# victorca25/traiNNer

Measured on NVIDIA B200. Metric: hr_pixels_per_sec, higher is better.
Workload: dtype bf16

## Files before the change

include/trainner_b200.h:

```cpp
#ifndef TRAINNER_B200_H_
#define TRAINNER_B200_H_

#include <stddef.h>
#include <stdint.h>

#ifdef __cplusplus
extern "C" {
#endif

typedef void* b200_stream_t;

#define B200_MAX_TAPS 16

typedef struct {
  int32_t n, h_in, w_in;
  int32_t cx, cin_off, cin;
  int32_t h_out, w_out;
  int32_t h_buf, w_buf, cy;
  int32_t cout_off, cout;
  int32_t ntaps;
  int8_t tap_dy[B200_MAX_TAPS], tap_dx[B200_MAX_TAPS], tap_w[B200_MAX_TAPS];
  int32_t in_stride, in_off_y, in_off_x;
  int32_t out_mul_y, out_off_y, out_mul_x, out_off_x;
  int32_t upsample2x;
  int32_t w_taps, w_cout_pad, w_cin_pad;
  float alpha;
  int32_t act;
  float slope;
  float beta1, beta2;
  int32_t res_nch;
  int32_t res1_c, res1_coff, res2_c, res2_coff;
  int32_t accumulate;
  int32_t mask_c, mask_coff, mask_lo, mask_hi;
  float mask_slope;
  int32_t parity_classes;
} b200_conv_desc;

int b200_conv_igemm(const b200_conv_desc* d, const void* x, const void* w_packed, const float* bias,
                    const void* res1, const void* res2, const void* mask, void* y,
                    b200_stream_t stream);
int b200_conv_igemm_stat_rows(const b200_conv_desc* d);
int b200_conv_igemm_stats(const b200_conv_desc* d, const void* x, const void* w_packed, const float* bias,
                          void* y, float* stat_part, b200_stream_t stream);

typedef struct {
  int32_t n, h, w;
  int32_t cx, cin_off, cin;
  int32_t cx2, cin2_off, cin2;
  int32_t cy, cout_off, cout;
  int8_t tap_dy[9], tap_dx[9], tap_w[9];
  int32_t out_mode;
  int32_t w_taps, w_cout_pad, w_cin_pad;
  float alpha;
  int32_t act;
  float slope;
  float beta1, beta2;
  int32_t res_nch, res1_c, res1_coff, res2_c, res2_coff;
  int32_t accumulate;
  int32_t mask_c, mask_coff, mask_lo, mask_hi;
  float mask_slope;
} b200_flat_desc;

int b200_conv3x3_flat(const b200_flat_desc* d, const void* x, const void* x2, const void* w_packed,
                      const float* bias, const void* res1, const void* res2, const void* mask, void* y,
                      b200_stream_t stream);

int b200_pad_copy(void* dst_flat, int32_t dst_c, int32_t dst_coff, const void* src_dense, int32_t src_c,
                  int32_t src_coff, int32_t n, int32_t h, int32_t w, int32_t c, b200_stream_t stream);
int b200_unpad_add(void* dst_dense, int32_t dst_c, const void* src_flat, int32_t src_c, int32_t src_coff,
                   const void* add_dense, int32_t add_c, int32_t n, int32_t h, int32_t w, int32_t c,
                   b200_stream_t stream);

typedef struct {
  void* out;
  const float* bias;
  const void* mask;
  const void* res1;
  const void* res2;
  int32_t out_c, out_coff, mask_c, mask_coff, res1_c, res1_coff, res2_c, res2_coff;
  float alpha, beta1, beta2, slope, mask_slope;
  int32_t act;
  int32_t pad_[2];
} b200_chain_stage;

typedef struct {
  int32_t n_total, img0, n;
  int32_t h, w;
  int32_t cx, x_coff;
  int32_t n_blocks;
  int32_t flip_taps;
} b200_chain_desc;

int b200_rdb_chain_geometry(int32_t n, int32_t h, int32_t w, int32_t* n_cta, int64_t* ll_bytes);
int b200_rdb_chain(const b200_chain_desc* d, const void* x0, const void* const* w_stage,
                   const b200_chain_stage* table_dev, void* ll_buf, int64_t ll_bytes, uint32_t* epoch_dev,
                   b200_stream_t stream);

typedef struct {
  int32_t n, h_in, w_in, cx, x_coff, cin;
  int32_t h_out, w_out, cdy, dy_coff, cout;
  int32_t kh, kw, stride, pad;
  float scale;
} b200_wgrad_desc;

int b200_conv_wgrad(const b200_wgrad_desc* d, const void* x, const void* dy, float* dw,
                    float* dbias, b200_stream_t stream);

typedef struct {
  float* dw[5];
  float scale5;
  int32_t pad_;
} b200_wgrad_rdb_entry;

int b200_tensor_map_bytes(void);
int b200_wgrad_rdb_make_maps(void* maps_host, int32_t n_rdb, const void* const* x_ptrs,
                             const void* const* g_ptrs, const void* const* do_ptrs,
                             const int32_t* do_pitch, int32_t n, int32_t h, int32_t w, int32_t c);
int64_t b200_wgrad_rdb_ws_bytes(int32_t n_rdb, int32_t n, int32_t h, int32_t w);
int b200_wgrad_rdb(const void* maps_dev, const b200_wgrad_rdb_entry* entries_dev, int32_t n_rdb,
                   int32_t n, int32_t h, int32_t w, int32_t nf, int32_t gc, void* workspace,
                   int64_t ws_bytes, b200_stream_t stream);

typedef struct {
  const void* src;
  float* dst;
  int64_t npix;
  int32_t pitch, coff, c;
  float scale;
} b200_colsum_entry;

int b200_colsum_multi(const b200_colsum_entry* table_dev, int32_t count, b200_stream_t stream);

typedef struct {
  const float* src;
  void* dst;
  int32_t cout, cin, taps, rows_pad, cols_pad, mode;
  int32_t co_mul, co_off;
} b200_pack_entry;

int b200_pack_weights(const b200_pack_entry* table_dev, int32_t count, int32_t max_elems,
                      b200_stream_t stream);

typedef struct {
  const float* src;
  void* dst;
  int32_t cout, cin, taps, ci_off, n_rows, rows_pad, cols_pad, col_off;
  float scale;
  int32_t row_off;
  int32_t mode;
  int32_t pad_;
} b200_packcat_entry;

int b200_pack_cat(const b200_packcat_entry* table_dev, int32_t count, int32_t max_elems,
                  b200_stream_t stream);

int b200_conv3x3_thin_to_wide(const float* x, const float* w_oihw, const float* bias, void* y,
                              int32_t n, int32_t h, int32_t w, int32_t cs, int32_t cw, int32_t cy,
                              int32_t y_coff, int32_t transpose_w, const float* mean,
                              const float* std, int32_t act, float slope, const void* mask,
                              int32_t mask_c, int32_t mask_coff, float mask_slope,
                              b200_stream_t stream);
int b200_conv3x3_wide_to_thin(const void* x, const float* w_oihw, const float* bias, float* y,
                              int32_t n, int32_t h, int32_t w, int32_t cw, int32_t cx, int32_t x_coff,
                              int32_t cs, int32_t transpose_w, const float* inv_std, float out_scale,
                              b200_stream_t stream);
int b200_conv3x3_thin_wgrad(const float* thin, const void* wide, float* dw, float* dbias_wide,
                            float* dbias_thin, int32_t n, int32_t h, int32_t w, int32_t cs,
                            int32_t cw, int32_t cwide_buf, int32_t wide_coff, int32_t wide_is_out,
                            const float* mean, const float* std, b200_stream_t stream);

int b200_bn_stats_finalize(const void* z, float* stats, float* mean_invstd, float* running_mean,
                           float* running_var, int64_t npix, int32_t c, float momentum, float eps,
                           b200_stream_t stream);
typedef struct {
  const float* stats;
  float* mean_invstd;
  float* running_mean;
  float* running_var;
  int64_t npix;
  int32_t c;
  float momentum, eps;
  int32_t pad_;
} b200_bn_finalize_entry;
int b200_bn_finalize_multi(const b200_bn_finalize_entry* table_dev, int32_t count, int32_t c_max,
                           b200_stream_t stream);
int b200_bn_partials_finalize(const float* part, int32_t rows, float* stats, float* mean_invstd,
                              float* running_mean, float* running_var, int64_t npix, int32_t c, float momentum,
                              float eps, b200_stream_t stream);
int b200_bn_apply_lrelu(const void* z, const float* mean_invstd, const float* gamma,
                        const float* beta, void* a, int64_t npix, int32_t c, float slope,
                        b200_stream_t stream);
int b200_bn_bwd_reduce(const void* z, const void* da, const float* mean_invstd,
                       const float* gamma, const float* beta, float* sums, float* dgamma, float* dbeta,
                       int64_t npix, int32_t c, float slope, b200_stream_t stream);
int b200_bn_bwd_apply(const void* z, const void* da, const float* mean_invstd, const float* gamma,
                      const float* beta, const float* sums, void* dz, int64_t npix, int32_t c, float slope,
                      int32_t use_batch_stats, b200_stream_t stream);

int b200_maxpool2x2(const void* x, void* y, int32_t n, int32_t h, int32_t w, int32_t c,
                    b200_stream_t stream);
int b200_maxpool2x2_bwd(const void* x, const void* dy, void* dx, int32_t n, int32_t h, int32_t w,
                        int32_t c, b200_stream_t stream);

int b200_sumpool2x2_mask(const void* dy, const void* mask_up, void* dx, int32_t n, int32_t h,
                         int32_t w, int32_t c, float slope, b200_stream_t stream);
int b200_pixel_shuffle2(const void* z, void* out, int32_t n, int32_t h, int32_t w, int32_t c,
                        int32_t act, float slope, b200_stream_t stream);
int b200_pixel_unshuffle2(const void* dout, void* dz, int32_t n, int32_t h, int32_t w, int32_t c,
                          b200_stream_t stream);

int b200_l1_loss_f32(const float* a, const float* b, float* loss_out, float* grad_a, int64_t numel,
                     float weight, b200_stream_t stream);
int b200_l1_loss_bf16(const void* a, const void* b, float* loss_out, void* grad_a, int64_t numel,
                      float weight, b200_stream_t stream);

int b200_lrelu_mask_mul(const void* g, const void* y, void* out, int64_t numel, float slope,
                        b200_stream_t stream);
int b200_nchw_f32_to_nhwc_bf16(const float* x, void* y, int32_t n, int32_t c, int32_t h, int32_t w,
                               int32_t cy, int32_t y_coff, b200_stream_t stream);
int b200_nhwc_bf16_to_nchw_f32(const void* x, float* y, int32_t n, int32_t c, int32_t h, int32_t w,
                               int32_t cx, int32_t x_coff, b200_stream_t stream);

const char* b200_last_error(void);
int b200_version(void);
int b200_device_ok(void);
int64_t b200_launch_count(void);

#ifdef __cplusplus
}
#endif
#endif
```

trainner_b200/_lib.py:

```python
import ctypes as C
import os

_HERE = os.path.dirname(os.path.abspath(__file__))
LIB_PATH = os.path.join(_HERE, "libtrainner_b200.so")

MAX_TAPS = 16


class ConvDesc(C.Structure):
    _fields_ = [
        ("n", C.c_int32), ("h_in", C.c_int32), ("w_in", C.c_int32),
        ("cx", C.c_int32), ("cin_off", C.c_int32), ("cin", C.c_int32),
        ("h_out", C.c_int32), ("w_out", C.c_int32),
        ("h_buf", C.c_int32), ("w_buf", C.c_int32), ("cy", C.c_int32),
        ("cout_off", C.c_int32), ("cout", C.c_int32),
        ("ntaps", C.c_int32),
        ("tap_dy", C.c_int8 * MAX_TAPS), ("tap_dx", C.c_int8 * MAX_TAPS), ("tap_w", C.c_int8 * MAX_TAPS),
        ("in_stride", C.c_int32), ("in_off_y", C.c_int32), ("in_off_x", C.c_int32),
        ("out_mul_y", C.c_int32), ("out_off_y", C.c_int32), ("out_mul_x", C.c_int32), ("out_off_x", C.c_int32),
        ("upsample2x", C.c_int32),
        ("w_taps", C.c_int32), ("w_cout_pad", C.c_int32), ("w_cin_pad", C.c_int32),
        ("alpha", C.c_float), ("act", C.c_int32), ("slope", C.c_float),
        ("beta1", C.c_float), ("beta2", C.c_float),
        ("res_nch", C.c_int32),
        ("res1_c", C.c_int32), ("res1_coff", C.c_int32), ("res2_c", C.c_int32), ("res2_coff", C.c_int32),
        ("accumulate", C.c_int32),
        ("mask_c", C.c_int32), ("mask_coff", C.c_int32), ("mask_lo", C.c_int32), ("mask_hi", C.c_int32),
        ("mask_slope", C.c_float),
        ("parity_classes", C.c_int32),
    ]


class FlatDesc(C.Structure):
    _fields_ = [
        ("n", C.c_int32), ("h", C.c_int32), ("w", C.c_int32),
        ("cx", C.c_int32), ("cin_off", C.c_int32), ("cin", C.c_int32),
        ("cx2", C.c_int32), ("cin2_off", C.c_int32), ("cin2", C.c_int32),
        ("cy", C.c_int32), ("cout_off", C.c_int32), ("cout", C.c_int32),
        ("tap_dy", C.c_int8 * 9), ("tap_dx", C.c_int8 * 9), ("tap_w", C.c_int8 * 9),
        ("out_mode", C.c_int32),
        ("w_taps", C.c_int32), ("w_cout_pad", C.c_int32), ("w_cin_pad", C.c_int32),
        ("alpha", C.c_float), ("act", C.c_int32), ("slope", C.c_float),
        ("beta1", C.c_float), ("beta2", C.c_float),
        ("res_nch", C.c_int32), ("res1_c", C.c_int32), ("res1_coff", C.c_int32),
        ("res2_c", C.c_int32), ("res2_coff", C.c_int32),
        ("accumulate", C.c_int32),
        ("mask_c", C.c_int32), ("mask_coff", C.c_int32), ("mask_lo", C.c_int32), ("mask_hi", C.c_int32),
        ("mask_slope", C.c_float),
    ]


class WgradDesc(C.Structure):
    _fields_ = [
        ("n", C.c_int32), ("h_in", C.c_int32), ("w_in", C.c_int32), ("cx", C.c_int32),
        ("x_coff", C.c_int32), ("cin", C.c_int32),
        ("h_out", C.c_int32), ("w_out", C.c_int32), ("cdy", C.c_int32), ("dy_coff", C.c_int32),
        ("cout", C.c_int32),
        ("kh", C.c_int32), ("kw", C.c_int32), ("stride", C.c_int32), ("pad", C.c_int32),
        ("scale", C.c_float),
    ]


class WgradRdbEntry(C.Structure):
    _fields_ = [("dw", C.c_void_p * 5), ("scale5", C.c_float), ("pad_", C.c_int32)]


class ColsumEntry(C.Structure):
    _fields_ = [("src", C.c_void_p), ("dst", C.c_void_p), ("npix", C.c_int64),
                ("pitch", C.c_int32), ("coff", C.c_int32), ("c", C.c_int32), ("scale", C.c_float)]


class BnFinalizeEntry(C.Structure):
    _fields_ = [("stats", C.c_void_p), ("mean_invstd", C.c_void_p), ("running_mean", C.c_void_p),
                ("running_var", C.c_void_p), ("npix", C.c_int64), ("c", C.c_int32), ("momentum", C.c_float),
                ("eps", C.c_float), ("pad_", C.c_int32)]


class PackCatEntry(C.Structure):
    _fields_ = [("src", C.c_void_p), ("dst", C.c_void_p),
                ("cout", C.c_int32), ("cin", C.c_int32), ("taps", C.c_int32), ("ci_off", C.c_int32),
                ("n_rows", C.c_int32), ("rows_pad", C.c_int32), ("cols_pad", C.c_int32), ("col_off", C.c_int32),
                ("scale", C.c_float), ("row_off", C.c_int32), ("mode", C.c_int32), ("pad_", C.c_int32)]


class ChainStage(C.Structure):
    _fields_ = [("out", C.c_void_p), ("bias", C.c_void_p), ("mask", C.c_void_p), ("res1", C.c_void_p),
                ("res2", C.c_void_p),
                ("out_c", C.c_int32), ("out_coff", C.c_int32), ("mask_c", C.c_int32), ("mask_coff", C.c_int32),
                ("res1_c", C.c_int32), ("res1_coff", C.c_int32), ("res2_c", C.c_int32), ("res2_coff", C.c_int32),
                ("alpha", C.c_float), ("beta1", C.c_float), ("beta2", C.c_float), ("slope", C.c_float),
                ("mask_slope", C.c_float), ("act", C.c_int32), ("pad_", C.c_int32 * 2)]


class ChainDesc(C.Structure):
    _fields_ = [("n_total", C.c_int32), ("img0", C.c_int32), ("n", C.c_int32), ("h", C.c_int32), ("w", C.c_int32),
                ("cx", C.c_int32), ("x_coff", C.c_int32), ("n_blocks", C.c_int32), ("flip_taps", C.c_int32)]


class PackEntry(C.Structure):
    _fields_ = [
        ("src", C.c_void_p), ("dst", C.c_void_p),
        ("cout", C.c_int32), ("cin", C.c_int32), ("taps", C.c_int32),
        ("rows_pad", C.c_int32), ("cols_pad", C.c_int32), ("mode", C.c_int32),
        ("co_mul", C.c_int32), ("co_off", C.c_int32),
    ]


_P, _I, _L, _F = C.c_void_p, C.c_int32, C.c_int64, C.c_float

_SIGNATURES = {
    "b200_conv_igemm": [C.POINTER(ConvDesc), _P, _P, _P, _P, _P, _P, _P, _P],
    "b200_conv_igemm_stats": [_P, _P, _P, _P, _P, _P, _P],
    "b200_conv3x3_flat": [C.POINTER(FlatDesc), _P, _P, _P, _P, _P, _P, _P, _P, _P],
    "b200_pack_cat": [_P, _I, _I, _P],
    "b200_rdb_chain": [C.POINTER(ChainDesc), _P, _P, _P, _P, _L, _P, _P],
    "b200_rdb_chain_geometry": [_I, _I, _I, _P, _P],
    "b200_pad_copy": [_P, _I, _I, _P, _I, _I, _I, _I, _I, _I, _P],
    "b200_unpad_add": [_P, _I, _P, _I, _I, _P, _I, _I, _I, _I, _I, _P],
    "b200_conv_wgrad": [C.POINTER(WgradDesc), _P, _P, _P, _P, _P],
    "b200_wgrad_rdb_make_maps": [_P, _I, _P, _P, _P, _P, _I, _I, _I, _I],
    "b200_wgrad_rdb": [_P, _P, _I, _I, _I, _I, _I, _I, _P, _L, _P],
    "b200_colsum_multi": [_P, _I, _P],
    "b200_pack_weights": [_P, _I, _I, _P],
    "b200_conv3x3_thin_to_wide": [_P, _P, _P, _P, _I, _I, _I, _I, _I, _I, _I, _I, _P, _P, _I, _F,
                                  _P, _I, _I, _F, _P],
    "b200_conv3x3_wide_to_thin": [_P, _P, _P, _P, _I, _I, _I, _I, _I, _I, _I, _I, _P, _F, _P],
    "b200_conv3x3_thin_wgrad": [_P, _P, _P, _P, _P, _I, _I, _I, _I, _I, _I, _I, _I, _P, _P, _P],
    "b200_bn_stats_finalize": [_P, _P, _P, _P, _P, _L, _I, _F, _F, _P],
    "b200_bn_partials_finalize": [_P, _I, _P, _P, _P, _P, _L, _I, _F, _F, _P],
    "b200_bn_finalize_multi": [_P, _I, _I, _P],
    "b200_bn_apply_lrelu": [_P, _P, _P, _P, _P, _L, _I, _F, _P],
    "b200_bn_bwd_reduce": [_P, _P, _P, _P, _P, _P, _P, _P, _L, _I, _F, _P],
    "b200_bn_bwd_apply": [_P, _P, _P, _P, _P, _P, _P, _L, _I, _F, _I, _P],
    "b200_maxpool2x2": [_P, _P, _I, _I, _I, _I, _P],
    "b200_maxpool2x2_bwd": [_P, _P, _P, _I, _I, _I, _I, _P],
    "b200_sumpool2x2_mask": [_P, _P, _P, _I, _I, _I, _I, _F, _P],
    "b200_pixel_shuffle2": [_P, _P, _I, _I, _I, _I, _I, _F, _P],
    "b200_pixel_unshuffle2": [_P, _P, _I, _I, _I, _I, _P],
    "b200_l1_loss_f32": [_P, _P, _P, _P, _L, _F, _P],
    "b200_l1_loss_bf16": [_P, _P, _P, _P, _L, _F, _P],
    "b200_lrelu_mask_mul": [_P, _P, _P, _L, _F, _P],
    "b200_nchw_f32_to_nhwc_bf16": [_P, _P, _I, _I, _I, _I, _I, _I, _P],
    "b200_nhwc_bf16_to_nchw_f32": [_P, _P, _I, _I, _I, _I, _I, _I, _P],
}

EXPORTED_SYMBOLS = sorted(list(_SIGNATURES) + ["b200_last_error", "b200_version", "b200_device_ok",
                                                "b200_launch_count", "b200_tensor_map_bytes",
                                                "b200_wgrad_rdb_ws_bytes", "b200_conv_igemm_stat_rows"])


def _load():
    if not os.path.exists(LIB_PATH):
        raise RuntimeError(
            "trainner_b200: %s not found. Build it with `python -c 'import __graft_entry__ as g; "
            "g.build()'` (nvcc, sm_100a). There is no CPU / PyTorch fallback." % LIB_PATH)
    lib = C.CDLL(LIB_PATH)
    for name, args in _SIGNATURES.items():
        fn = getattr(lib, name)
        fn.argtypes = args
        fn.restype = C.c_int
    lib.b200_last_error.restype = C.c_char_p
    lib.b200_version.restype = C.c_int
    lib.b200_device_ok.restype = C.c_int
    lib.b200_launch_count.restype = C.c_int64
    lib.b200_tensor_map_bytes.restype = C.c_int
    lib.b200_tensor_map_bytes.argtypes = []
    lib.b200_conv_igemm_stat_rows.restype = C.c_int
    lib.b200_conv_igemm_stat_rows.argtypes = [C.POINTER(ConvDesc)]
    lib.b200_wgrad_rdb_ws_bytes.restype = C.c_int64
    lib.b200_wgrad_rdb_ws_bytes.argtypes = [_I, _I, _I, _I]
    return lib


lib = _load()


def check(rc, what=""):
    if rc != 0:
        raise RuntimeError("trainner_b200 %s failed: %s" % (what, lib.b200_last_error().decode()))


def launch_count():
    return int(lib.b200_launch_count())
```

trainner_b200/csrc/common.cu:

```cuda
#include "common.cuh"

#include <map>
#include <mutex>
#include <utility>
#include <stdlib.h>

namespace b200 {

thread_local char g_err[512] = {0};
std::atomic<long long> g_launches{0};

EncodeTiled_t get_encode_tiled() {
  static EncodeTiled_t fn = nullptr;
  static std::once_flag once;
  std::call_once(once, [] {
    void* p = nullptr;
    cudaDriverEntryPointQueryResult qr;
    if (cudaGetDriverEntryPoint("cuTensorMapEncodeTiled", &p, cudaEnableDefault, &qr) ==
            cudaSuccess &&
        qr == cudaDriverEntryPointSuccess)
      fn = reinterpret_cast<EncodeTiled_t>(p);
  });
  return fn;
}

bool pdl_enabled() {
  static int on = -1;
  if (on < 0) {
    const char* e = getenv("B200_PDL");
    on = (e && e[0] == '0') ? 0 : 1;
  }
  return on == 1;
}

int sm_count() {
  static std::mutex mu;
  static int cache[64] = {0};
  int dev = 0;
  if (cudaGetDevice(&dev) != cudaSuccess) return 148;
  std::lock_guard<std::mutex> g(mu);
  if (dev < 0 || dev >= 64) dev = 0;
  if (cache[dev] == 0) {
    int n = 0;
    cudaDeviceGetAttribute(&n, cudaDevAttrMultiProcessorCount, dev);
    cache[dev] = n > 0 ? n : 148;
  }
  return cache[dev];
}

int ensure_max_smem(const void* kernel, int bytes, bool prefer_max_carveout) {
  static std::mutex mu;
  static std::map<std::pair<const void*, int>, int> done;
  int dev = 0;
  cudaError_t e = cudaGetDevice(&dev);
  if (e != cudaSuccess) return set_error("cudaGetDevice failed: %s", cudaGetErrorString(e));
  std::lock_guard<std::mutex> g(mu);
  auto key = std::make_pair(kernel, dev);
  auto it = done.find(key);
  if (it != done.end() && it->second >= bytes) return 0;
  e = cudaFuncSetAttribute(kernel, cudaFuncAttributeMaxDynamicSharedMemorySize, bytes);
  if (e == cudaSuccess && prefer_max_carveout)
    e = cudaFuncSetAttribute(kernel, cudaFuncAttributePreferredSharedMemoryCarveout, cudaSharedmemCarveoutMaxShared);
  if (e != cudaSuccess)
    return set_error("cudaFuncSetAttribute(max dynamic smem %d) failed on device %d: %s", bytes, dev,
                     cudaGetErrorString(e));
  done[key] = bytes;
  return 0;
}

int det_scratch(DetScratch* out, size_t floats_needed, int counters_needed) {
  static std::mutex mu;
  static DetScratch per_dev[64] = {};
  if (floats_needed > kDetFloats || counters_needed > kDetCounters)
    return set_error("deterministic-reduction scratch too small: need %zu floats / %d counters", floats_needed,
                     counters_needed);
  int dev = 0;
  cudaError_t e = cudaGetDevice(&dev);
  if (e != cudaSuccess || dev < 0 || dev >= 64) return set_error("det_scratch: cudaGetDevice failed");
  std::lock_guard<std::mutex> g(mu);
  if (!per_dev[dev].part) {
    void* p = nullptr;
    e = cudaMalloc(&p, kDetFloats * sizeof(float) + kDetCounters * sizeof(unsigned));
    if (e != cudaSuccess)
      return set_error("det_scratch: cudaMalloc failed (%s) -- the first call of a reduction kernel must not happen "
                       "inside a stream capture", cudaGetErrorString(e));
    e = cudaMemset(static_cast<float*>(p) + kDetFloats, 0, kDetCounters * sizeof(unsigned));
    if (e != cudaSuccess) return set_error("det_scratch: cudaMemset failed (%s)", cudaGetErrorString(e));
    per_dev[dev].part = static_cast<float*>(p);
    per_dev[dev].counters = reinterpret_cast<unsigned*>(static_cast<float*>(p) + kDetFloats);
  }
  *out = per_dev[dev];
  return 0;
}

int make_tensor_map(CUtensorMap* m, const void* ptr, int rank, const uint64_t* dims,
                    const uint64_t* strides_bytes, const uint32_t* box,
                    const uint32_t* elem_strides, CUtensorMapSwizzle swizzle) {
  EncodeTiled_t enc = get_encode_tiled();
  if (!enc) return set_error("cuTensorMapEncodeTiled unavailable (no CUDA driver?)");
  cuuint64_t d[5], s[4];
  cuuint32_t b[5], e[5];
  for (int i = 0; i < rank; ++i) {
    d[i] = dims[i];
    b[i] = box[i];
    e[i] = elem_strides ? elem_strides[i] : 1;
    if (i < rank - 1) s[i] = strides_bytes[i];
  }
  CUresult r = enc(m, CU_TENSOR_MAP_DATA_TYPE_BFLOAT16, rank, const_cast<void*>(ptr), d, s, b, e,
                   CU_TENSOR_MAP_INTERLEAVE_NONE, swizzle, CU_TENSOR_MAP_L2_PROMOTION_L2_256B,
                   CU_TENSOR_MAP_FLOAT_OOB_FILL_NONE);
  if (r != CUDA_SUCCESS) {
    return set_error(
        "cuTensorMapEncodeTiled failed (%d): rank %d dims [%llu %llu %llu %llu] box [%u %u %u %u] "
        "stride0 %llu ptr %p",
        (int)r, rank, (unsigned long long)d[0], (unsigned long long)(rank > 1 ? d[1] : 0),
        (unsigned long long)(rank > 2 ? d[2] : 0), (unsigned long long)(rank > 3 ? d[3] : 0), b[0],
        rank > 1 ? b[1] : 0, rank > 2 ? b[2] : 0, rank > 3 ? b[3] : 0,
        (unsigned long long)(rank > 1 ? s[0] : 0), ptr);
  }
  return 0;
}

}

extern "C" {

const char* b200_last_error(void) { return b200::g_err; }
int b200_version(void) { return 100; }
int64_t b200_launch_count(void) { return b200::g_launches.load(); }
int b200_device_ok(void) {
  int dev = 0;
  if (cudaGetDevice(&dev) != cudaSuccess) return 0;
  int major = 0;
  if (cudaDeviceGetAttribute(&major, cudaDevAttrComputeCapabilityMajor, dev) != cudaSuccess) return 0;
  return major == 10 ? 1 : 0;
}
}
```

trainner_b200/csrc/common.cuh:

```cuda
#pragma once
#include <cuda.h>
#include <cuda_bf16.h>
#include <cuda_runtime.h>
#include <stdarg.h>
#include <stdint.h>
#include <stdio.h>

#include <atomic>

#include "../../include/trainner_b200.h"

namespace b200 {

extern thread_local char g_err[512];
extern std::atomic<long long> g_launches;

inline int set_error(const char* fmt, ...) {
  va_list ap;
  va_start(ap, fmt);
  vsnprintf(g_err, sizeof(g_err), fmt, ap);
  va_end(ap);
  return 1;
}

#define B200_CHECK_CUDA(expr)                                                               \
  do {                                                                                      \
    cudaError_t e_ = (expr);                                                                \
    if (e_ != cudaSuccess)                                                                  \
      return ::b200::set_error("%s failed: %s (%s:%d)", #expr, cudaGetErrorString(e_), __FILE__, \
                               __LINE__);                                                   \
  } while (0)

#define B200_REQUIRE(cond, ...)                      \
  do {                                               \
    if (!(cond)) return ::b200::set_error(__VA_ARGS__); \
  } while (0)

#define B200_LAUNCH_CHECK()                \
  do {                                     \
    ::b200::g_launches.fetch_add(1);       \
    B200_CHECK_CUDA(cudaGetLastError());   \
  } while (0)

typedef CUresult (*EncodeTiled_t)(CUtensorMap*, CUtensorMapDataType, cuuint32_t, void*,
                                  const cuuint64_t*, const cuuint64_t*, const cuuint32_t*,
                                  const cuuint32_t*, CUtensorMapInterleave, CUtensorMapSwizzle,
                                  CUtensorMapL2promotion, CUtensorMapFloatOOBfill);
EncodeTiled_t get_encode_tiled();
int sm_count();

int ensure_max_smem(const void* kernel, int bytes, bool prefer_max_carveout = false);
#define B200_ENSURE_SMEM(kernel, bytes) \
  do { if (::b200::ensure_max_smem(reinterpret_cast<const void*>(kernel), (bytes))) return 1; } while (0)

int make_tensor_map(CUtensorMap* m, const void* ptr, int rank, const uint64_t* dims,
                    const uint64_t* strides_bytes, const uint32_t* box, const uint32_t* elem_strides,
                    CUtensorMapSwizzle swizzle);

struct DetScratch {
  float* part;
  unsigned* counters;
};
constexpr size_t kDetFloats = 16u << 20;
constexpr int kDetCounters = 8192;
int det_scratch(DetScratch* out, size_t floats_needed, int counters_needed);

inline cudaStream_t as_stream(b200_stream_t s) { return reinterpret_cast<cudaStream_t>(s); }

bool pdl_enabled();

template <typename... KArgs, typename... Args>
inline cudaError_t launch_kernel(void (*kernel)(KArgs...), dim3 grid, dim3 block, size_t smem,
                                 cudaStream_t stream, Args&&... args) {
  cudaLaunchConfig_t cfg = {};
  cfg.gridDim = grid;
  cfg.blockDim = block;
  cfg.dynamicSmemBytes = smem;
  cfg.stream = stream;
  cudaLaunchAttribute attr[1];
  attr[0].id = cudaLaunchAttributeProgrammaticStreamSerialization;
  attr[0].val.programmaticStreamSerializationAllowed = 1;
  cfg.attrs = attr;
  cfg.numAttrs = pdl_enabled() ? 1 : 0;
  return cudaLaunchKernelEx(&cfg, kernel, static_cast<KArgs>(args)...);
}

#ifdef __CUDACC__
__device__ __forceinline__ void pdl_trigger() { asm volatile("griddepcontrol.launch_dependents;" ::: "memory"); }
__device__ __forceinline__ void pdl_wait() { asm volatile("griddepcontrol.wait;" ::: "memory"); }

__device__ __forceinline__ bool det_arrive_last(unsigned* counter, unsigned nblk) {
  __shared__ unsigned s_last;
  __threadfence();
  __syncthreads();
  if (threadIdx.x == 0 && threadIdx.y == 0 && threadIdx.z == 0) {
    const unsigned t = atomicAdd(counter, 1u);
    s_last = (t == nblk - 1) ? 1u : 0u;
    if (s_last) *counter = 0u;
  }
  __syncthreads();
  const bool last = s_last != 0u;
  if (last) __threadfence();
  return last;
}

constexpr int kDetGroup = 16;
__host__ __device__ __forceinline__ int det_groups(int nblk) { return (nblk + kDetGroup - 1) / kDetGroup; }

template <typename F>
__device__ __forceinline__ bool det_reduce(const float* __restrict__ part, float* __restrict__ gpart,
                                           unsigned* counters, unsigned nblk, int nout, F&& out) {
  const unsigned grp = blockIdx.x / kDetGroup, ngrp = det_groups((int)nblk);
  const unsigned g0 = grp * kDetGroup;
  const unsigned members = (nblk - g0) < (unsigned)kDetGroup ? (nblk - g0) : (unsigned)kDetGroup;
  if (!det_arrive_last(counters + 1 + grp, members)) return false;
  for (int k = threadIdx.x; k < nout; k += blockDim.x) {
    const float* row = part + (size_t)k * nblk + g0;
    float t = 0.f;
#pragma unroll 4
    for (unsigned i = 0; i < members; ++i) t += row[i];
    gpart[(size_t)k * ngrp + grp] = t;
  }
  if (!det_arrive_last(counters, ngrp)) return false;
  for (int k = threadIdx.x; k < nout; k += blockDim.x) {
    const float* row = gpart + (size_t)k * ngrp;
    float t = 0.f;
#pragma unroll 4
    for (unsigned g = 0; g < ngrp; ++g) t += row[g];
    out(k, t);
  }
  return true;
}
#endif

}
```

trainner_b200/csrc/elementwise.cu:

```cuda
#include "common.cuh"

namespace b200 {
namespace {

__device__ __forceinline__ void unpack8(const uint4& u, float* f) {
  const __nv_bfloat162* h = reinterpret_cast<const __nv_bfloat162*>(&u);
#pragma unroll
  for (int i = 0; i < 4; ++i) {
    float2 t = __bfloat1622float2(h[i]);
    f[2 * i] = t.x;
    f[2 * i + 1] = t.y;
  }
}
__device__ __forceinline__ uint4 pack8(const float* f) {
  uint4 u;
  __nv_bfloat162* h = reinterpret_cast<__nv_bfloat162*>(&u);
#pragma unroll
  for (int i = 0; i < 4; ++i) h[i] = __floats2bfloat162_rn(f[2 * i], f[2 * i + 1]);
  return u;
}
__device__ __forceinline__ float warp_sum(float v) {
#pragma unroll
  for (int o = 16; o > 0; o >>= 1) v += __shfl_xor_sync(0xffffffffu, v, o);
  return v;
}

inline int grid_for(long long work_items, int threads, int max_blocks = 148 * 16) {
  long long b = (work_items + threads - 1) / threads;
  if (b < 1) b = 1;
  if (b > max_blocks) b = max_blocks;
  return (int)b;
}

__device__ __forceinline__ void bn_finalize_channel(const float* stats, float* mean_invstd, float* running_mean,
                                                    float* running_var, long long npix, int c, float momentum,
                                                    float eps, int ch) {
  const double n = (double)npix;
  const double mean = stats[ch] / n;
  double var = stats[c + ch] / n - mean * mean;
  if (var < 0) var = 0;
  mean_invstd[ch] = (float)mean;
  mean_invstd[c + ch] = (float)(1.0 / sqrt(var + (double)eps));
  if (running_mean) {
    const double unbiased = npix > 1 ? var * n / (n - 1.0) : var;
    running_mean[ch] = (float)((1.0 - momentum) * running_mean[ch] + momentum * mean);
    running_var[ch] = (float)((1.0 - momentum) * running_var[ch] + momentum * unbiased);
  }
}

template <int MODE>
__global__ void bn_reduce_kernel(const __nv_bfloat16* __restrict__ z,
                                 const __nv_bfloat16* __restrict__ da,
                                 const float* __restrict__ mean_invstd,
                                 const float* __restrict__ gamma, const float* __restrict__ beta,
                                 float* __restrict__ sums, long long npix, int c, float slope,
                                 float* __restrict__ part, unsigned* __restrict__ counter,
                                 float* __restrict__ dgamma, float* __restrict__ dbeta,
                                 float* __restrict__ fin_mean_invstd, float* __restrict__ running_mean,
                                 float* __restrict__ running_var, float momentum, float eps) {
  pdl_trigger();
  pdl_wait();
  const int vec_per_pix = c / 8;
  const long long total_vec = npix * vec_per_pix;
  const long long stride = (long long)gridDim.x * blockDim.x;
  long long i = (long long)blockIdx.x * blockDim.x + threadIdx.x;
  const int cv = (int)(i % vec_per_pix) * 8;
  float s0[8], s1[8];
#pragma unroll
  for (int j = 0; j < 8; ++j) s0[j] = s1[j] = 0.f;
  float mu[8], is[8], ga[8], be[8];
  if (MODE == 1) {
#pragma unroll
    for (int j = 0; j < 8; ++j) {
      mu[j] = mean_invstd[cv + j];
      is[j] = mean_invstd[c + cv + j];
      ga[j] = gamma[cv + j];
      be[j] = beta[cv + j];
    }
  }
  constexpr int U = 4;
  for (; i < total_vec; i += U * stride) {
    uint4 zv[U], gv[U];
#pragma unroll
    for (int u = 0; u < U; ++u) {
      const long long iu = i + u * stride;
      zv[u] = iu < total_vec ? reinterpret_cast<const uint4*>(z)[iu] : make_uint4(0, 0, 0, 0);
      if (MODE == 1) gv[u] = iu < total_vec ? reinterpret_cast<const uint4*>(da)[iu] : make_uint4(0, 0, 0, 0);
    }
#pragma unroll
    for (int u = 0; u < U; ++u) {
      if (i + u * stride >= total_vec) break;
      float f[8];
      unpack8(zv[u], f);
      if (MODE == 0) {
#pragma unroll
        for (int j = 0; j < 8; ++j) {
          s0[j] += f[j];
          s1[j] = fmaf(f[j], f[j], s1[j]);
        }
      } else {
        float g[8];
        unpack8(gv[u], g);
#pragma unroll
        for (int j = 0; j < 8; ++j) {
          const float zh = (f[j] - mu[j]) * is[j];
          const float bn = fmaf(ga[j], zh, be[j]);
          const float d = bn > 0.f ? g[j] : g[j] * slope;
          s0[j] += d;
          s1[j] = fmaf(d, zh, s1[j]);
        }
      }
    }
  }
  extern __shared__ float sh[];
#pragma unroll
  for (int j = 0; j < 8; ++j) {
    sh[j * 256 + threadIdx.x] = s0[j];
    sh[(8 + j) * 256 + threadIdx.x] = s1[j];
  }
  __syncthreads();
  for (int k = threadIdx.x; k < 2 * c; k += blockDim.x) {
    const int which = k / c, ch = k - which * c;
    const int ln = ch >> 3, j = (ch & 7) + 8 * which;
    float t = 0.f;
    for (int q = ln; q < 256; q += vec_per_pix) t += sh[j * 256 + q];
    part[(size_t)k * gridDim.x + blockIdx.x] = t;
  }
  const bool fin = det_reduce(part, part + (size_t)2 * c * gridDim.x, counter, gridDim.x, 2 * c, [&](int k, float t) {
    sums[k] = t;
    if (MODE == 1) {
      if (k < c) {
        if (dbeta) dbeta[k] += t;
      } else if (dgamma) {
        dgamma[k - c] += t;
      }
    }
  });
  if (MODE == 0 && fin && fin_mean_invstd) {
    __syncthreads();
    for (int ch = threadIdx.x; ch < c; ch += blockDim.x)
      bn_finalize_channel(sums, fin_mean_invstd, running_mean, running_var, npix, c, momentum, eps, ch);
  }
}

__global__ void bn_finalize_multi_kernel(const b200_bn_finalize_entry* __restrict__ table) {
  pdl_trigger();
  pdl_wait();
  const b200_bn_finalize_entry e = table[blockIdx.y];
  const int ch = blockIdx.x * blockDim.x + threadIdx.x;
  if (ch >= e.c) return;
  bn_finalize_channel(e.stats, e.mean_invstd, e.running_mean, e.running_var, e.npix, e.c, e.momentum, e.eps, ch);
}

__global__ void __launch_bounds__(256) bn_partials_finalize_kernel(const float* __restrict__ part, int rows,
                                                                   float* __restrict__ stats,
                                                                   float* __restrict__ mean_invstd,
                                                                   float* __restrict__ running_mean,
                                                                   float* __restrict__ running_var, long long npix, int c,
                                                                   float momentum, float eps) {
  pdl_trigger();
  pdl_wait();
  const int lane = threadIdx.x & 31, ch = blockIdx.x * 8 + (threadIdx.x >> 5);
  if (ch >= c) return;
  float s0 = 0.f, s1 = 0.f;
  const float* p0 = part + (size_t)ch * rows;
  const float* p1 = part + (size_t)(c + ch) * rows;
  for (int i = lane; i < rows; i += 32) {
    s0 += p0[i];
    s1 += p1[i];
  }
#pragma unroll
  for (int o = 16; o > 0; o >>= 1) {
    s0 += __shfl_xor_sync(0xffffffffu, s0, o);
    s1 += __shfl_xor_sync(0xffffffffu, s1, o);
  }
  if (lane == 0) {
    stats[ch] = s0;
    stats[c + ch] = s1;
    bn_finalize_channel(stats, mean_invstd, running_mean, running_var, npix, c, momentum, eps, ch);
  }
}

template <int MODE>
__global__ void bn_apply_kernel(const __nv_bfloat16* __restrict__ z,
                                const __nv_bfloat16* __restrict__ da,
                                const float* __restrict__ mean_invstd,
                                const float* __restrict__ gamma, const float* __restrict__ beta,
                                const float* __restrict__ sums, __nv_bfloat16* __restrict__ out,
                                long long npix, int c, float slope, int use_batch_stats) {
  pdl_trigger();
  pdl_wait();
  const int vec_per_pix = c / 8;
  const long long total_vec = npix * vec_per_pix;
  const long long stride = (long long)gridDim.x * blockDim.x;
  long long i = (long long)blockIdx.x * blockDim.x + threadIdx.x;
  const int cv = (int)(i % vec_per_pix) * 8;
  float mu[8], is[8], ga[8], be[8], m0[8], m1[8];
  const float inv_n = use_batch_stats ? 1.f / (float)npix : 0.f;
#pragma unroll
  for (int j = 0; j < 8; ++j) {
    mu[j] = mean_invstd[cv + j];
    is[j] = mean_invstd[c + cv + j];
    ga[j] = gamma[cv + j];
    be[j] = beta[cv + j];
    if (MODE == 1) {
      m0[j] = sums[cv + j] * inv_n;
      m1[j] = sums[c + cv + j] * inv_n;
    }
  }
  constexpr int U = 2;
  for (; i < total_vec; i += U * stride) {
    uint4 zv[U], gv[U];
#pragma unroll
    for (int u = 0; u < U; ++u) {
      const long long iu = i + u * stride;
      zv[u] = iu < total_vec ? reinterpret_cast<const uint4*>(z)[iu] : make_uint4(0, 0, 0, 0);
      if (MODE == 1) gv[u] = iu < total_vec ? reinterpret_cast<const uint4*>(da)[iu] : make_uint4(0, 0, 0, 0);
    }
#pragma unroll
    for (int u = 0; u < U; ++u) {
      const long long iu = i + u * stride;
      if (iu >= total_vec) break;
      float f[8], o[8];
      unpack8(zv[u], f);
      if (MODE == 0) {
#pragma unroll
        for (int j = 0; j < 8; ++j) {
          const float bn = fmaf(ga[j], (f[j] - mu[j]) * is[j], be[j]);
          o[j] = bn > 0.f ? bn : bn * slope;
        }
      } else {
        float g[8];
        unpack8(gv[u], g);
#pragma unroll
        for (int j = 0; j < 8; ++j) {
          const float zh = (f[j] - mu[j]) * is[j];
          const float bn = fmaf(ga[j], zh, be[j]);
          const float d = bn > 0.f ? g[j] : g[j] * slope;
          o[j] = ga[j] * is[j] * (d - m0[j] - zh * m1[j]);
        }
      }
      reinterpret_cast<uint4*>(out)[iu] = pack8(o);
    }
  }
}

__global__ void add_small_kernel(float* __restrict__ dst, const float* __restrict__ src, int n) {
  pdl_trigger();
  pdl_wait();
  const int i = blockIdx.x * blockDim.x + threadIdx.x;
  if (i < n) dst[i] += src[i];
}

template <int BWD>
__global__ void pixel_shuffle2_kernel(const __nv_bfloat16* __restrict__ src, __nv_bfloat16* __restrict__ dst,
                                      int n, int h, int w, int c, int act, float slope) {
  pdl_trigger();
  pdl_wait();
  const int qn = c / 8;
  const long long total = (long long)n * h * w * qn;
  for (long long idx = (long long)blockIdx.x * blockDim.x + threadIdx.x; idx < total;
       idx += (long long)gridDim.x * blockDim.x) {
    const int q = (int)(idx % qn);
    long long r = idx / qn;
    const int x = (int)(r % w);
    r /= w;
    const int y = (int)(r % h);
    const int b = (int)(r / h);
    const long long zoff = ((((long long)b * h + y) * w + x) * 4 * c) + 32 * q;
    float v[32];
    if (BWD == 0) {
#pragma unroll
      for (int u = 0; u < 4; ++u) unpack8(*reinterpret_cast<const uint4*>(src + zoff + 8 * u), v + 8 * u);
    }
#pragma unroll
    for (int k = 0; k < 4; ++k) {
      const long long ooff = ((((long long)b * 2 * h + 2 * y + (k >> 1)) * 2 * w + 2 * x + (k & 1)) * c) + 8 * q;
      float o[8];
      if (BWD == 0) {
#pragma unroll
        for (int cc = 0; cc < 8; ++cc) {
          const float t = v[cc * 4 + k];
          o[cc] = (act && t < 0.f) ? t * slope : t;
        }
        *reinterpret_cast<uint4*>(dst + ooff) = pack8(o);
      } else {
        unpack8(*reinterpret_cast<const uint4*>(src + ooff), o);
#pragma unroll
        for (int cc = 0; cc < 8; ++cc) v[cc * 4 + k] = o[cc];
      }
    }
    if (BWD == 1) {
#pragma unroll
      for (int u = 0; u < 4; ++u) *reinterpret_cast<uint4*>(dst + zoff + 8 * u) = pack8(v + 8 * u);
    }
  }
}

__global__ void maxpool_kernel(const __nv_bfloat16* __restrict__ x, __nv_bfloat16* __restrict__ y,
                               int n, int h, int w, int c) {
  pdl_trigger();
  pdl_wait();
  const int ho = h / 2, wo = w / 2, cv = c / 8;
  const long long total = (long long)n * ho * wo * cv;
  for (long long i = (long long)blockIdx.x * blockDim.x + threadIdx.x; i < total;
       i += (long long)gridDim.x * blockDim.x) {
    const int v = (int)(i % cv);
    long long r = i / cv;
    const int xo = (int)(r % wo);
    r /= wo;
    const int yo = (int)(r % ho);
    const int b = (int)(r / ho);
    const uint4* base = reinterpret_cast<const uint4*>(x) +
                        (((long long)b * h + 2 * yo) * w + 2 * xo) * cv + v;
    float a[8], t[8];
    unpack8(base[0], a);
    unpack8(base[cv], t);
#pragma unroll
    for (int j = 0; j < 8; ++j) a[j] = t[j] > a[j] ? t[j] : a[j];
    unpack8(base[(long long)w * cv], t);
#pragma unroll
    for (int j = 0; j < 8; ++j) a[j] = t[j] > a[j] ? t[j] : a[j];
    unpack8(base[(long long)w * cv + cv], t);
#pragma unroll
    for (int j = 0; j < 8; ++j) a[j] = t[j] > a[j] ? t[j] : a[j];
    reinterpret_cast<uint4*>(y)[i] = pack8(a);
  }
}

__global__ void maxpool_bwd_kernel(const __nv_bfloat16* __restrict__ x,
                                   const __nv_bfloat16* __restrict__ dy,
                                   __nv_bfloat16* __restrict__ dx, int n, int h, int w, int c) {
  pdl_trigger();
  pdl_wait();
  const int ho = h / 2, wo = w / 2, cv = c / 8;
  const long long total = (long long)n * ho * wo * cv;
  for (long long i = (long long)blockIdx.x * blockDim.x + threadIdx.x; i < total;
       i += (long long)gridDim.x * blockDim.x) {
    const int v = (int)(i % cv);
    long long r = i / cv;
    const int xo = (int)(r % wo);
    r /= wo;
    const int yo = (int)(r % ho);
    const int b = (int)(r / ho);
    const long long o00 = (((long long)b * h + 2 * yo) * w + 2 * xo) * cv + v;
    const long long offs[4] = {o00, o00 + cv, o00 + (long long)w * cv, o00 + (long long)w * cv + cv};
    float q[4][8], g[8];
#pragma unroll
    for (int k = 0; k < 4; ++k) unpack8(reinterpret_cast<const uint4*>(x)[offs[k]], q[k]);
    unpack8(reinterpret_cast<const uint4*>(dy)[i], g);
    float o[4][8];
#pragma unroll
    for (int j = 0; j < 8; ++j) {
      int arg = 0;
      float best = q[0][j];
#pragma unroll
      for (int k = 1; k < 4; ++k)
        if (q[k][j] > best) {
          best = q[k][j];
          arg = k;
        }
#pragma unroll
      for (int k = 0; k < 4; ++k) o[k][j] = (k == arg && best > 0.f) ? g[j] : 0.f;
    }
#pragma unroll
    for (int k = 0; k < 4; ++k) reinterpret_cast<uint4*>(dx)[offs[k]] = pack8(o[k]);
  }
}

__global__ void sumpool_mask_kernel(const __nv_bfloat16* __restrict__ dy,
                                    const __nv_bfloat16* __restrict__ mask,
                                    __nv_bfloat16* __restrict__ dx, int n, int h, int w, int c,
                                    float slope) {
  pdl_trigger();
  pdl_wait();
  const int cv = c / 8;
  const long long total = (long long)n * h * w * cv;
  for (long long i = (long long)blockIdx.x * blockDim.x + threadIdx.x; i < total;
       i += (long long)gridDim.x * blockDim.x) {
    const int v = (int)(i % cv);
    long long r = i / cv;
    const int xo = (int)(r % w);
    r /= w;
    const int yo = (int)(r % h);
    const int b = (int)(r / h);
    const long long o00 = (((long long)b * 2 * h + 2 * yo) * 2 * w + 2 * xo) * cv + v;
    float a[8], t[8];
    unpack8(reinterpret_cast<const uint4*>(dy)[o00], a);
    unpack8(reinterpret_cast<const uint4*>(dy)[o00 + cv], t);
#pragma unroll
    for (int j = 0; j < 8; ++j) a[j] += t[j];
    unpack8(reinterpret_cast<const uint4*>(dy)[o00 + (long long)2 * w * cv], t);
#pragma unroll
    for (int j = 0; j < 8; ++j) a[j] += t[j];
    unpack8(reinterpret_cast<const uint4*>(dy)[o00 + (long long)2 * w * cv + cv], t);
#pragma unroll
    for (int j = 0; j < 8; ++j) a[j] += t[j];
    if (mask) {
      unpack8(reinterpret_cast<const uint4*>(mask)[o00], t);
#pragma unroll
      for (int j = 0; j < 8; ++j) a[j] = t[j] > 0.f ? a[j] : a[j] * slope;
    }
    reinterpret_cast<uint4*>(dx)[i] = pack8(a);
  }
}

__global__ void lrelu_mask_mul_kernel(const __nv_bfloat16* __restrict__ g,
                                      const __nv_bfloat16* __restrict__ y,
                                      __nv_bfloat16* __restrict__ out, long long nvec, float slope) {
  pdl_trigger();
  pdl_wait();
  for (long long i = (long long)blockIdx.x * blockDim.x + threadIdx.x; i < nvec;
       i += (long long)gridDim.x * blockDim.x) {
    float a[8], t[8];
    unpack8(reinterpret_cast<const uint4*>(g)[i], a);
    unpack8(reinterpret_cast<const uint4*>(y)[i], t);
#pragma unroll
    for (int j = 0; j < 8; ++j) a[j] = t[j] > 0.f ? a[j] : a[j] * slope;
    reinterpret_cast<uint4*>(out)[i] = pack8(a);
  }
}

template <typename T>
__device__ __forceinline__ float ld_as_float(const T* p, long long i);
template <>
__device__ __forceinline__ float ld_as_float<float>(const float* p, long long i) { return p[i]; }
template <>
__device__ __forceinline__ float ld_as_float<__nv_bfloat16>(const __nv_bfloat16* p, long long i) {
  return __bfloat162float(p[i]);
}
__device__ __forceinline__ void st_from_float(float* p, long long i, float v) { p[i] = v; }
__device__ __forceinline__ void st_from_float(__nv_bfloat16* p, long long i, float v) {
  p[i] = __float2bfloat16(v);
}

template <typename T>
__global__ void l1_loss_kernel(const T* __restrict__ a, const T* __restrict__ b,
                               float* __restrict__ loss_out, T* __restrict__ grad_a, long long numel,
                               float scale, float* __restrict__ part, unsigned* __restrict__ counter) {
  pdl_trigger();
  pdl_wait();
  float s = 0.f;
  for (long long i = (long long)blockIdx.x * blockDim.x + threadIdx.x; i < numel;
       i += (long long)gridDim.x * blockDim.x) {
    const float d = ld_as_float(a, i) - ld_as_float(b, i);
    s += fabsf(d);
    if (grad_a) st_from_float(grad_a, i, d > 0.f ? scale : (d < 0.f ? -scale : 0.f));
  }
  s = warp_sum(s);
  __shared__ float red[32];
  const int w = threadIdx.x >> 5, l = threadIdx.x & 31;
  if (l == 0) red[w] = s;
  __syncthreads();
  if (w == 0) {
    s = l < (blockDim.x >> 5) ? red[l] : 0.f;
    s = warp_sum(s);
    if (l == 0) part[blockIdx.x] = s;
  }
  det_reduce(part, part + gridDim.x, counter, gridDim.x, 1, [&](int, float t) { *loss_out = t * scale; });
}

__global__ void nchw_to_nhwc_kernel(const float* __restrict__ x, __nv_bfloat16* __restrict__ y, int n,
                                    int c, int h, int w, int cy, int coff) {
  pdl_trigger();
  pdl_wait();
  const long long hw = (long long)h * w;
  const long long total = (long long)n * hw * c;
  for (long long i = (long long)blockIdx.x * blockDim.x + threadIdx.x; i < total;
       i += (long long)gridDim.x * blockDim.x) {
    const int ch = (int)(i % c);
    const long long pix = i / c;
    const long long b = pix / hw, p = pix % hw;
    y[pix * cy + coff + ch] = __float2bfloat16(x[(b * c + ch) * hw + p]);
  }
}
__global__ void nhwc_to_nchw_kernel(const __nv_bfloat16* __restrict__ x, float* __restrict__ y, int n,
                                    int c, int h, int w, int cx, int coff) {
  pdl_trigger();
  pdl_wait();
  const long long total = (long long)n * c * h * w;
  for (long long i = (long long)blockIdx.x * blockDim.x + threadIdx.x; i < total;
       i += (long long)gridDim.x * blockDim.x) {
    const long long hw = i % ((long long)h * w);
    const long long r = i / ((long long)h * w);
    const int ch = (int)(r % c);
    const long long b = r / c;
    y[i] = __bfloat162float(x[(b * h * w + hw) * cx + coff + ch]);
  }
}
inline int bn_grid(long long npix, int c, int per_thread, int max_blocks = 148 * 8) {
  const int vpp = c / 8;
  long long total = (npix * vpp + per_thread - 1) / per_thread;
  int g = grid_for(total, 256, max_blocks);
  while ((256LL * g) % vpp != 0) ++g;
  return g;
}

}
}

using namespace b200;
typedef __nv_bfloat16 bf16;

extern "C" {

int b200_bn_stats_finalize(const void* z, float* stats, float* mean_invstd, float* running_mean,
                           float* running_var, int64_t npix, int32_t c, float momentum, float eps,
                           b200_stream_t stream) {
  B200_REQUIRE(mean_invstd != nullptr, "b200_bn_stats_finalize: mean_invstd is required");
  B200_REQUIRE(c % 8 == 0 && c <= 2048 && 256 % (c / 8) == 0,
               "b200_bn_stats_finalize: c/8 must be a power of two <= 256 (c=%d)", c);
  const int grid = bn_grid(npix, c, 4, 148 * 2);
  DetScratch ds;
  if (det_scratch(&ds, (size_t)(grid + det_groups(grid)) * 2 * c, 1 + det_groups(grid))) return 1;
  ::b200::launch_kernel(bn_reduce_kernel<0>, grid, 256, 16 * 256 * sizeof(float), as_stream(stream),
      (const bf16*)z, nullptr, nullptr, nullptr, nullptr, stats, (long long)npix, c, 0.f, ds.part, ds.counters, nullptr, nullptr,
      mean_invstd, running_mean, running_var, momentum, eps);
  B200_LAUNCH_CHECK();
  return 0;
}

int b200_bn_finalize_multi(const b200_bn_finalize_entry* table_dev, int32_t count, int32_t c_max,
                           b200_stream_t stream) {
  if (count <= 0) return 0;
  B200_REQUIRE(table_dev && c_max > 0, "b200_bn_finalize_multi: bad arguments");
  ::b200::launch_kernel(bn_finalize_multi_kernel, dim3((c_max + 127) / 128, count), 128, 0, as_stream(stream), table_dev);
  B200_LAUNCH_CHECK();
  return 0;
}

int b200_bn_partials_finalize(const float* part, int32_t rows, float* stats, float* mean_invstd,
                              float* running_mean, float* running_var, int64_t npix, int32_t c, float momentum,
                              float eps, b200_stream_t stream) {
  B200_REQUIRE(part && stats && mean_invstd && rows > 0, "b200_bn_partials_finalize: bad arguments");
  ::b200::launch_kernel(bn_partials_finalize_kernel, (c + 7) / 8, 256, 0, as_stream(stream),
      part, (int)rows, stats, mean_invstd, running_mean, running_var, (long long)npix, (int)c, momentum, eps);
  B200_LAUNCH_CHECK();
  return 0;
}

int b200_bn_apply_lrelu(const void* z, const float* mean_invstd, const float* gamma,
                        const float* beta, void* a, int64_t npix, int32_t c, float slope,
                        b200_stream_t stream) {
  B200_REQUIRE(c % 8 == 0, "b200_bn_apply_lrelu: c must be a multiple of 8");
  ::b200::launch_kernel(bn_apply_kernel<0>, bn_grid(npix, c, 2), 256, 0, as_stream(stream), 
      (const bf16*)z, nullptr, mean_invstd, gamma, beta, nullptr, (bf16*)a, npix, c, slope, 1);
  B200_LAUNCH_CHECK();
  return 0;
}

int b200_bn_bwd_reduce(const void* z, const void* da, const float* mean_invstd, const float* gamma,
                       const float* beta, float* sums, float* dgamma, float* dbeta, int64_t npix, int32_t c,
                       float slope, b200_stream_t stream) {
  B200_REQUIRE(c % 8 == 0 && c <= 2048 && 256 % (c / 8) == 0, "b200_bn_bwd_reduce: c/8 must be a power of two <= 256 (c=%d)", c);
  const int grid = bn_grid(npix, c, 4, 148 * 2);
  DetScratch ds;
  if (det_scratch(&ds, (size_t)(grid + det_groups(grid)) * 2 * c, 1 + det_groups(grid))) return 1;
  ::b200::launch_kernel(bn_reduce_kernel<1>, grid, 256, 16 * 256 * sizeof(float), as_stream(stream), 
      (const bf16*)z, (const bf16*)da, mean_invstd, gamma, beta, sums, npix, c, slope, ds.part, ds.counters, dgamma, dbeta,
      nullptr, nullptr, nullptr, 0.f, 0.f);
  B200_LAUNCH_CHECK();
  return 0;
}

int b200_bn_bwd_apply(const void* z, const void* da, const float* mean_invstd, const float* gamma,
                      const float* beta, const float* sums, void* dz, int64_t npix, int32_t c, float slope,
                      int32_t use_batch_stats, b200_stream_t stream) {
  ::b200::launch_kernel(bn_apply_kernel<1>, bn_grid(npix, c, 2), 256, 0, as_stream(stream), 
      (const bf16*)z, (const bf16*)da, mean_invstd, gamma, beta, sums, (bf16*)dz, npix, c, slope, (int)use_batch_stats);
  B200_LAUNCH_CHECK();
  return 0;
}

int b200_maxpool2x2(const void* x, void* y, int32_t n, int32_t h, int32_t w, int32_t c,
                    b200_stream_t stream) {
  B200_REQUIRE(c % 8 == 0 && h % 2 == 0 && w % 2 == 0, "b200_maxpool2x2: bad shape");
  const long long total = (long long)n * (h / 2) * (w / 2) * (c / 8);
  ::b200::launch_kernel(maxpool_kernel, grid_for(total, 256), 256, 0, as_stream(stream), (const bf16*)x, (bf16*)y, n, h,
                                                                     w, c);
  B200_LAUNCH_CHECK();
  return 0;
}

int b200_maxpool2x2_bwd(const void* x, const void* dy, void* dx, int32_t n, int32_t h, int32_t w,
                        int32_t c, b200_stream_t stream) {
  B200_REQUIRE(c % 8 == 0 && h % 2 == 0 && w % 2 == 0, "b200_maxpool2x2_bwd: bad shape");
  const long long total = (long long)n * (h / 2) * (w / 2) * (c / 8);
  ::b200::launch_kernel(maxpool_bwd_kernel, grid_for(total, 256), 256, 0, as_stream(stream), 
      (const bf16*)x, (const bf16*)dy, (bf16*)dx, n, h, w, c);
  B200_LAUNCH_CHECK();
  return 0;
}

int b200_sumpool2x2_mask(const void* dy, const void* mask, void* dx, int32_t n, int32_t h,
                         int32_t w, int32_t c, float slope, b200_stream_t stream) {
  B200_REQUIRE(c % 8 == 0, "b200_sumpool2x2_mask: bad shape");
  const long long total = (long long)n * h * w * (c / 8);
  ::b200::launch_kernel(sumpool_mask_kernel, grid_for(total, 256), 256, 0, as_stream(stream), 
      (const bf16*)dy, (const bf16*)mask, (bf16*)dx, n, h, w, c, slope);
  B200_LAUNCH_CHECK();
  return 0;
}

int b200_pixel_shuffle2(const void* z, void* out, int32_t n, int32_t h, int32_t w, int32_t c, int32_t act,
                        float slope, b200_stream_t stream) {
  B200_REQUIRE(z && out && c % 8 == 0, "b200_pixel_shuffle2: c (output channels) must be a multiple of 8");
  const long long total = (long long)n * h * w * (c / 8);
  ::b200::launch_kernel(pixel_shuffle2_kernel<0>, grid_for(total, 256), 256, 0, as_stream(stream),
                        (const bf16*)z, (bf16*)out, n, h, w, c, act, slope);
  B200_LAUNCH_CHECK();
  return 0;
}

int b200_pixel_unshuffle2(const void* dout, void* dz, int32_t n, int32_t h, int32_t w, int32_t c,
                          b200_stream_t stream) {
  B200_REQUIRE(dout && dz && c % 8 == 0, "b200_pixel_unshuffle2: c (output channels) must be a multiple of 8");
  const long long total = (long long)n * h * w * (c / 8);
  ::b200::launch_kernel(pixel_shuffle2_kernel<1>, grid_for(total, 256), 256, 0, as_stream(stream),
                        (const bf16*)dout, (bf16*)dz, n, h, w, c, 0, 0.f);
  B200_LAUNCH_CHECK();
  return 0;
}

int b200_l1_loss_f32(const float* a, const float* b, float* loss_out, float* grad_a, int64_t numel,
                     float weight, b200_stream_t stream) {
  const int grid = grid_for(numel, 256, 148 * 4);
  DetScratch ds;
  if (det_scratch(&ds, (size_t)grid + det_groups(grid), 1 + det_groups(grid))) return 1;
  ::b200::launch_kernel(l1_loss_kernel<float>, grid, 256, 0, as_stream(stream), 
      a, b, loss_out, grad_a, numel, weight / (float)numel, ds.part, ds.counters);
  B200_LAUNCH_CHECK();
  return 0;
}

int b200_l1_loss_bf16(const void* a, const void* b, float* loss_out, void* grad_a, int64_t numel,
                      float weight, b200_stream_t stream) {
  const int grid = grid_for(numel, 256, 148 * 4);
  DetScratch ds;
  if (det_scratch(&ds, (size_t)grid + det_groups(grid), 1 + det_groups(grid))) return 1;
  ::b200::launch_kernel(l1_loss_kernel<bf16>, grid, 256, 0, as_stream(stream), 
      (const bf16*)a, (const bf16*)b, loss_out, (bf16*)grad_a, numel, weight / (float)numel, ds.part, ds.counters);
  B200_LAUNCH_CHECK();
  return 0;
}

int b200_lrelu_mask_mul(const void* g, const void* y, void* out, int64_t numel, float slope,
                        b200_stream_t stream) {
  B200_REQUIRE(numel % 8 == 0, "b200_lrelu_mask_mul: numel must be a multiple of 8");
  ::b200::launch_kernel(lrelu_mask_mul_kernel, grid_for(numel / 8, 256), 256, 0, as_stream(stream), 
      (const bf16*)g, (const bf16*)y, (bf16*)out, numel / 8, slope);
  B200_LAUNCH_CHECK();
  return 0;
}

int b200_nchw_f32_to_nhwc_bf16(const float* x, void* y, int32_t n, int32_t c, int32_t h, int32_t w,
                               int32_t cy, int32_t y_coff, b200_stream_t stream) {
  ::b200::launch_kernel(nchw_to_nhwc_kernel, grid_for((long long)n * h * w * c, 256), 256, 0, as_stream(stream), 
      x, (bf16*)y, n, c, h, w, cy, y_coff);
  B200_LAUNCH_CHECK();
  return 0;
}

int b200_nhwc_bf16_to_nchw_f32(const void* x, float* y, int32_t n, int32_t c, int32_t h, int32_t w,
                               int32_t cx, int32_t x_coff, b200_stream_t stream) {
  ::b200::launch_kernel(nhwc_to_nchw_kernel, grid_for((long long)n * c * h * w, 256), 256, 0, as_stream(stream), 
      (const bf16*)x, y, n, c, h, w, cx, x_coff);
  B200_LAUNCH_CHECK();
  return 0;
}

}
```

trainner_b200/engine_d.py:

```python
import weakref

import torch

from ._lib import BnFinalizeEntry, lib
from .runtime import (ConvLayer, ContextPool, pool_for, FlatGrads, Lease, LRELU_SLOPE, P, Plan, WeightPacker,
                      add_igemm, add_igemm_stats, igemm_stat_rows, add_wgrad, make_conv_desc, require_device, taps_conv, taps_dgrad_s1,
                      taps_dgrad_s2_k4)

BF16 = torch.bfloat16


class _DContext:
    pass


class DiscriminatorEngine:
    def __init__(self, net):
        self.net = net
        self.device = None
        self.pools = {}
        self.reuse = False
        self._cache = {}

    def _setup(self, device):
        net = self.net
        self.device = device
        feats = list(net.features)
        self.conv0 = feats[0]
        self.layers = []
        i = 2
        while i < len(feats):
            conv, bn = feats[i], feats[i + 1]
            assert isinstance(conv, torch.nn.Conv2d) and isinstance(bn, torch.nn.BatchNorm2d)
            self.layers.append((ConvLayer(conv, "features.%d" % i), bn))
            i += 3
        self.packer = WeightPacker([l for l, _ in self.layers], device)
        self.grads = FlatGrads(list(net.features.parameters()), device)
        self.pools = {}

    def _ensure(self, x):
        require_device(x, "Discriminator_VGG")
        if self.device != x.device or self.packer.stale_pointers():
            self._setup(x.device)

    def _make_context(self, N, S):
        net = self.net
        dev = self.device
        ctx = _DContext()
        ctx.N, ctx.S = N, S
        e = lambda *s: torch.empty(*s, dtype=BF16, device=dev)
        c0 = self.conv0.out_channels
        ctx.x = torch.empty(N, net.in_nc, S, S, dtype=torch.float32, device=dev)
        ctx.A = [e(N, S, S, c0)]
        ctx.Z, ctx.stats, ctx.mi, ctx.dims = [], [], [], []
        ctx.stat_part = [None] * len(self.layers)
        h = S
        for L, bn in self.layers:
            ho = (h + 2 * L.pad - L.kh) // L.stride + 1
            ctx.Z.append(e(N, ho, ho, L.cout))
            ctx.A.append(e(N, ho, ho, L.cout))
            ctx.stats.append(torch.empty(2 * L.cout, dtype=torch.float32, device=dev))
            ctx.mi.append(torch.empty(2 * L.cout, dtype=torch.float32, device=dev))
            ctx.dims.append((h, ho))
            h = ho
        ctx.hf = h
        cl = self.layers[-1][0].cout if self.layers else c0
        ctx.feat = torch.empty(N, cl, h, h, dtype=torch.float32, device=dev)
        SL = LRELU_SLOPE

        def fwd_plan(train):
            f = Plan()
            f.add(lib.b200_conv3x3_thin_to_wide, P(ctx.x), P(self.conv0.weight), P(self.conv0.bias), P(ctx.A[0]),
                  N, S, S, net.in_nc, c0, c0, 0, 0, None, None, 1, SL, None, 0, 0, 0.0)
            for i, (L, bn) in enumerate(self.layers):
                hi, ho = ctx.dims[i]
                d = make_conv_desc(N, hi, hi, L.cin, 0, L.cin, ho, ho, ho, ho, L.cout, 0, L.cout,
                                   taps_conv(L.kh, L.pad), L.taps, L.fwd_rows, L.fwd_cols, in_stride=L.stride)
                npix = N * ho * ho
                rows = igemm_stat_rows(d) if train else 0
                if rows:
                    if ctx.stat_part[i] is None:
                        ctx.stat_part[i] = torch.empty(2 * L.cout * rows, dtype=torch.float32, device=dev)
                    add_igemm_stats(f, d, ctx.A[i], L.w_fwd, L.bias, ctx.Z[i], ctx.stat_part[i])
                    f.add(lib.b200_bn_partials_finalize, P(ctx.stat_part[i]), rows, P(ctx.stats[i]), P(ctx.mi[i]),
                          P(bn.running_mean), P(bn.running_var), npix, L.cout, float(bn.momentum), float(bn.eps))
                else:
                    add_igemm(f, d, ctx.A[i], L.w_fwd, L.bias, y=ctx.Z[i])
                if train and not rows:
                    f.add(lib.b200_bn_stats_finalize, P(ctx.Z[i]), P(ctx.stats[i]), P(ctx.mi[i]),
                          P(bn.running_mean), P(bn.running_var), npix, L.cout, float(bn.momentum), float(bn.eps))
                f.add(lib.b200_bn_apply_lrelu, P(ctx.Z[i]), P(ctx.mi[i]), P(bn.weight), P(bn.bias),
                      P(ctx.A[i + 1]), npix, L.cout, SL)
            f.add(lib.b200_nhwc_bf16_to_nchw_f32, P(ctx.A[-1]), P(ctx.feat), N, cl, ctx.hf, ctx.hf, cl, 0)
            return f

        ctx.fwd_train = fwd_plan(True)
        ctx.fwd_eval = fwd_plan(False)
        rf = Plan()
        ents = [BnFinalizeEntry(ctx.stats[i].data_ptr(), ctx.mi[i].data_ptr(), bn.running_mean.data_ptr(),
                                bn.running_var.data_ptr(), N * ctx.dims[i][1] * ctx.dims[i][1], L.cout,
                                float(bn.momentum), float(bn.eps), 0) for i, (L, bn) in enumerate(self.layers)]
        ctx.refinalize_table = torch.frombuffer(bytearray(bytes((BnFinalizeEntry * len(ents))(*ents))),
                                                dtype=torch.uint8).to(dev)
        rf.add(lib.b200_bn_finalize_multi, P(ctx.refinalize_table), len(ents), max(L.cout for L, _ in self.layers))
        ctx.refinalize = rf
        ctx.bwd = {}
        return ctx

    def _make_backward(self, ctx, wgrad, xgrad, train=True):
        net = self.net
        dev = self.device
        N, S = ctx.N, ctx.S
        SL = LRELU_SLOPE
        g = self.grads.view
        e = lambda *s: torch.empty(*s, dtype=BF16, device=dev)
        if not hasattr(ctx, "dA"):
            ctx.dfeat = torch.empty_like(ctx.feat)
            ctx.dA = [e(*a.shape) for a in ctx.A]
            ctx.dZ = [e(*z.shape) for z in ctx.Z]
            ctx.sums = [torch.empty_like(s) for s in ctx.stats]
            ctx.dx = torch.empty_like(ctx.x)
        b = Plan()
        cl = ctx.feat.shape[1]
        b.add(lib.b200_nchw_f32_to_nhwc_bf16, P(ctx.dfeat), P(ctx.dA[-1]), N, cl, ctx.hf, ctx.hf, cl, 0)
        c0 = self.conv0.out_channels
        for i in range(len(self.layers) - 1, -1, -1):
            L, bn = self.layers[i]
            hi, ho = ctx.dims[i]
            npix = N * ho * ho
            b.add(lib.b200_bn_bwd_reduce, P(ctx.Z[i]), P(ctx.dA[i + 1]), P(ctx.mi[i]), P(bn.weight), P(bn.bias),
                  P(ctx.sums[i]), P(g(bn.weight)) if wgrad else None, P(g(bn.bias)) if wgrad else None, npix, L.cout,
                  SL)
            b.add(lib.b200_bn_bwd_apply, P(ctx.Z[i]), P(ctx.dA[i + 1]), P(ctx.mi[i]), P(bn.weight), P(bn.bias),
                  P(ctx.sums[i]), P(ctx.dZ[i]), npix, L.cout, SL, 1 if train else 0)
            if wgrad:
                add_wgrad(b, N, hi, hi, L.cin, 0, L.cin, ho, ho, L.cout, 0, L.cout, L.kh, L.stride, L.pad, 1.0,
                          ctx.A[i], ctx.dZ[i], g(L.weight), g(L.bias))
            if i == 0 and not (wgrad or xgrad):
                break
            mask_kw = dict(mask_c=c0, mask_coff=0, mask_lo=0, mask_hi=c0, mask_slope=SL) if i == 0 else {}
            mask_t = ctx.A[0] if i == 0 else None
            if L.stride == 1:
                d = make_conv_desc(N, ho, ho, L.cout, 0, L.cout, hi, hi, hi, hi, L.cin, 0, L.cin,
                                   taps_dgrad_s1(L.kh, L.pad), L.taps, L.dgr_rows, L.dgr_cols, **mask_kw)
                add_igemm(b, d, ctx.dZ[i], L.w_dgr, mask=mask_t, y=ctx.dA[i])
            else:
                assert L.stride == 2 and L.kh == 4 and L.pad == 1
                taps4 = [t for py in (0, 1) for px in (0, 1) for t in taps_dgrad_s2_k4(py, px)]
                d = make_conv_desc(N, ho, ho, L.cout, 0, L.cout, hi // 2, hi // 2, hi, hi, L.cin, 0, L.cin,
                                   taps4, L.taps, L.dgr_rows, L.dgr_cols, out_mul=(2, 2), out_off=(0, 0),
                                   parity_classes=4, **mask_kw)
                add_igemm(b, d, ctx.dZ[i], L.w_dgr, mask=mask_t, y=ctx.dA[i])
        if wgrad:
            b.add(lib.b200_conv3x3_thin_wgrad, P(ctx.x), P(ctx.dA[0]), P(g(self.conv0.weight)),
                  P(g(self.conv0.bias)), None, N, S, S, net.in_nc, c0, c0, 0, 1, None, None)
        if xgrad:
            b.add(lib.b200_conv3x3_wide_to_thin, P(ctx.dA[0]), P(self.conv0.weight), None, P(ctx.dx), N, S, S, c0,
                  c0, 0, net.in_nc, 1, None, 1.0)
        ctx.bwd[(wgrad, xgrad, train)] = b

    def forward(self, x, need_backward, training):
        self._ensure(x)
        N, _, S, S2 = x.shape
        if S != S2:
            raise RuntimeError("Discriminator_VGG expects square inputs, got %dx%d" % (S, S2))
        key = (N, S)
        pool = pool_for(self.pools, key, lambda: self._make_context(N, S))
        self.packer.ensure()
        ckey = (x.data_ptr(), x._version, tuple(x.shape))
        if self.reuse and training:
            hit = self._cache.get(ckey)
            if hit is not None and hit[1] == self.packer.pack_count and hit[0] in pool.free \
                    and hit[2]() is not None:
                ctx = hit[0]
                pool.free.remove(ctx)
                ctx.refinalize.run()
                for _, bn in self.layers:
                    bn.num_batches_tracked.add_(1)
                feat = ctx.feat.clone()
                if need_backward:
                    return feat, Lease(pool, ctx)
                pool.release(ctx)
                return feat, None
        ctx = pool.acquire()
        for k in [k for k, v in self._cache.items() if v[0] is ctx]:
            del self._cache[k]
        if self.reuse and training:
            self._cache[ckey] = (ctx, self.packer.pack_count, weakref.ref(x))
        ctx.x.copy_(x)
        ctx.trained = bool(training)
        if training:
            ctx.fwd_train.run()
            for _, bn in self.layers:
                bn.num_batches_tracked.add_(1)
        else:
            for i, (L, bn) in enumerate(self.layers):
                ctx.mi[i][:L.cout].copy_(bn.running_mean)
                ctx.mi[i][L.cout:].copy_(torch.rsqrt(bn.running_var + bn.eps))
            ctx.fwd_eval.run()
        feat = ctx.feat.clone()
        if need_backward:
            return feat, Lease(pool, ctx)
        pool.release(ctx)
        return feat, None

    def backward(self, lease, dfeat, xgrad):
        ctx = lease.ctx
        wgrad = any(p.requires_grad for p in self.net.features.parameters())
        key = (wgrad, xgrad, bool(ctx.trained))
        if key not in ctx.bwd:
            self._make_backward(ctx, wgrad, xgrad, train=bool(ctx.trained))
        if wgrad:
            self.grads.attach()
        ctx.dfeat.copy_(dfeat)
        ctx.bwd[key].run()
        dx = ctx.dx.clone() if xgrad else None
        lease.release()
        return dx
```

trainner_b200/ops.py:

```python
import ctypes as C

import torch

from . import _lib
from ._lib import PackEntry, WgradDesc, lib
from .runtime import (make_conv_desc, make_flat_desc, require_device, roundup, stream_ptr, taps_conv, taps_dgrad_s1,
                      taps_dgrad_s2_k4)

BF16 = torch.bfloat16


def _p(t):
    return None if t is None else t.data_ptr()


def pack_weight(w_oihw, mode, co_mul=0, co_off=0, cout=None):
    require_device(w_oihw, "pack_weight")
    w = w_oihw.detach().float().contiguous()
    co, ci, kh, kw = w.shape
    if cout is not None:
        co = cout
    taps = kh * kw
    rows, cols = (roundup(co, 16), roundup(ci, 64)) if mode == 0 else (roundup(ci, 16), roundup(co, 64))
    dst = torch.empty(taps, rows, cols, dtype=BF16, device=w.device)
    e = PackEntry(w.data_ptr(), dst.data_ptr(), co, ci, taps, rows, cols, mode, co_mul, co_off)
    table = torch.frombuffer(bytearray(bytes(e)), dtype=torch.uint8).to(w.device)
    _lib.check(lib.b200_pack_weights(table.data_ptr(), 1, taps * rows * cols, stream_ptr()), "pack_weights")
    return dst


def conv2d(x, w_oihw, bias=None, stride=1, padding=1, cin_off=0, cin=None, out=None, cout_off=0, act=0,
           slope=0.2, alpha=1.0, res1=None, res1_coff=0, beta1=0.0, res2=None, res2_coff=0, beta2=0.0,
           res_nch=0, upsample2x=False):
    require_device(x, "conv2d")
    N, H, W, Cx = x.shape
    Cout, Cin, kh, kw = w_oihw.shape
    cin = Cin if cin is None else cin
    assert cin == Cin
    Ho = (H + 2 * padding - kh) // stride + 1
    Wo = (W + 2 * padding - kw) // stride + 1
    Hb, Wb = (2 * Ho, 2 * Wo) if upsample2x else (Ho, Wo)
    if out is None:
        out = torch.empty(N, Hb, Wb, Cout, dtype=BF16, device=x.device)
    wp = pack_weight(w_oihw, 0)
    d = make_conv_desc(N, H, W, Cx, cin_off, cin, Ho, Wo, Hb, Wb, out.shape[3], cout_off, Cout,
                       taps_conv(kh, padding), kh * kw, wp.shape[1], wp.shape[2], in_stride=stride,
                       upsample=1 if upsample2x else 0, alpha=alpha, act=act, slope=slope, beta1=beta1,
                       beta2=beta2, res_nch=res_nch,
                       res1_c=res1.shape[3] if res1 is not None else 0, res1_coff=res1_coff,
                       res2_c=res2.shape[3] if res2 is not None else 0, res2_coff=res2_coff)
    b = bias.detach().float().contiguous() if bias is not None else None
    _lib.check(lib.b200_conv_igemm(C.byref(d), _p(x), _p(wp), _p(b), _p(res1), _p(res2), None, _p(out),
                                   stream_ptr()), "conv_igemm")
    return out


def conv2d_dgrad(dy, w_oihw, in_hw, stride=1, padding=1, dy_coff=0, out=None, dx_coff=0, alpha=1.0,
                 accumulate=False, mask=None, mask_coff=0, mask_lo=0, mask_hi=0, mask_slope=0.2, res1=None,
                 res1_coff=0, beta1=0.0, res_nch=0):
    require_device(dy, "conv2d_dgrad")
    N, Ho, Wo, Cdy = dy.shape
    Cout, Cin, kh, kw = w_oihw.shape
    H, W = in_hw
    if out is None:
        out = torch.zeros(N, H, W, Cin, dtype=BF16, device=dy.device)
    wp = pack_weight(w_oihw, 1)
    common = dict(alpha=alpha, accumulate=1 if accumulate else 0,
                  mask_c=mask.shape[3] if mask is not None else 0, mask_coff=mask_coff, mask_lo=mask_lo,
                  mask_hi=mask_hi, mask_slope=mask_slope, beta1=beta1, res_nch=res_nch,
                  res1_c=res1.shape[3] if res1 is not None else 0, res1_coff=res1_coff)
    descs = []
    if stride == 1:
        descs.append(make_conv_desc(N, Ho, Wo, Cdy, dy_coff, Cout, H, W, H, W, out.shape[3], dx_coff, Cin,
                                    taps_dgrad_s1(kh, padding), kh * kw, wp.shape[1], wp.shape[2], **common))
    else:
        assert stride == 2 and kh == 4 and padding == 1 and H % 2 == 0 and W % 2 == 0
        for py in (0, 1):
            for px in (0, 1):
                descs.append(make_conv_desc(N, Ho, Wo, Cdy, dy_coff, Cout, H // 2, W // 2, H, W, out.shape[3],
                                            dx_coff, Cin, taps_dgrad_s2_k4(py, px), 16, wp.shape[1],
                                            wp.shape[2], out_mul=(2, 2), out_off=(py, px), **common))
    for d in descs:
        _lib.check(lib.b200_conv_igemm(C.byref(d), _p(dy), _p(wp), None, _p(res1), None, _p(mask), _p(out),
                                       stream_ptr()), "conv_igemm(dgrad)")
    return out


def conv2d_wgrad(x, dy, w_shape, stride=1, padding=1, x_coff=0, dy_coff=0, scale=1.0, want_bias=True):
    require_device(x, "conv2d_wgrad")
    N, H, W, Cx = x.shape
    _, Ho, Wo, Cdy = dy.shape
    Cout, Cin, kh, kw = w_shape
    dw = torch.zeros(w_shape, dtype=torch.float32, device=x.device)
    db = torch.zeros(Cout, dtype=torch.float32, device=x.device) if want_bias else None
    d = WgradDesc(N, H, W, Cx, x_coff, Cin, Ho, Wo, Cdy, dy_coff, Cout, kh, kw, stride, padding, scale)
    _lib.check(lib.b200_conv_wgrad(C.byref(d), _p(x), _p(dy), _p(dw), _p(db), stream_ptr()), "conv_wgrad")
    return dw, db


def conv3x3_thin_to_wide(x, w, bias=None, transpose_w=False, cw=None, mean=None, std=None, act=0, slope=0.2,
                         mask=None, mask_slope=0.2):
    require_device(x, "conv3x3_thin_to_wide")
    N, cs, H, W = x.shape
    cw = (w.shape[1] if transpose_w else w.shape[0]) if cw is None else cw
    y = torch.empty(N, H, W, cw, dtype=BF16, device=x.device)
    _lib.check(lib.b200_conv3x3_thin_to_wide(_p(x), _p(w), _p(bias), _p(y), N, H, W, cs, cw, cw, 0,
                                             1 if transpose_w else 0, _p(mean), _p(std), act, slope, _p(mask),
                                             mask.shape[3] if mask is not None else 0, 0, mask_slope,
                                             stream_ptr()), "thin_to_wide")
    return y


def conv3x3_wide_to_thin(x, w, bias=None, transpose_w=False, cs=None, inv_std=None, out_scale=1.0):
    require_device(x, "conv3x3_wide_to_thin")
    N, H, W, cw = x.shape
    cs = (w.shape[1] if transpose_w else w.shape[0]) if cs is None else cs
    y = torch.empty(N, cs, H, W, dtype=torch.float32, device=x.device)
    _lib.check(lib.b200_conv3x3_wide_to_thin(_p(x), _p(w), _p(bias), _p(y), N, H, W, cw, cw, 0, cs,
                                             1 if transpose_w else 0, _p(inv_std), out_scale, stream_ptr()),
               "wide_to_thin")
    return y


def conv3x3_thin_wgrad(thin, wide, wide_is_out, want_bias_wide=False, want_bias_thin=False):
    require_device(thin, "conv3x3_thin_wgrad")
    N, cs, H, W = thin.shape
    cw = wide.shape[3]
    shape = (cw, cs, 3, 3) if wide_is_out else (cs, cw, 3, 3)
    dw = torch.zeros(shape, dtype=torch.float32, device=thin.device)
    dbw = torch.zeros(cw, dtype=torch.float32, device=thin.device) if want_bias_wide else None
    dbt = torch.zeros(cs, dtype=torch.float32, device=thin.device) if want_bias_thin else None
    _lib.check(lib.b200_conv3x3_thin_wgrad(_p(thin), _p(wide), _p(dw), _p(dbw), _p(dbt), N, H, W, cs, cw, cw, 0,
                                           1 if wide_is_out else 0, None, None, stream_ptr()), "thin_wgrad")
    return dw, dbw, dbt


def batchnorm_lrelu_train(z, gamma, beta, running_mean=None, running_var=None, momentum=0.1, eps=1e-5,
                          slope=0.2):
    require_device(z, "batchnorm_lrelu_train")
    c = z.shape[-1]
    npix = z.numel() // c
    stats = torch.empty(2 * c, dtype=torch.float32, device=z.device)
    mi = torch.empty(2 * c, dtype=torch.float32, device=z.device)
    a = torch.empty_like(z)
    s = stream_ptr()
    _lib.check(lib.b200_bn_stats_finalize(_p(z), _p(stats), _p(mi), _p(running_mean), _p(running_var), npix, c,
                                          momentum, eps, s), "bn_stats_finalize")
    _lib.check(lib.b200_bn_apply_lrelu(_p(z), _p(mi), _p(gamma), _p(beta), _p(a), npix, c, slope, s), "bn_apply")
    return a, mi


def batchnorm_lrelu_backward(z, da, mi, gamma, beta, slope=0.2, use_batch_stats=True):
    require_device(z, "batchnorm_lrelu_backward")
    c = z.shape[-1]
    npix = z.numel() // c
    sums = torch.empty(2 * c, dtype=torch.float32, device=z.device)
    dz = torch.empty_like(z)
    dgamma = torch.zeros(c, dtype=torch.float32, device=z.device)
    dbeta = torch.zeros(c, dtype=torch.float32, device=z.device)
    s = stream_ptr()
    _lib.check(lib.b200_bn_bwd_reduce(_p(z), _p(da), _p(mi), _p(gamma), _p(beta), _p(sums), _p(dgamma), _p(dbeta), npix,
                                      c, slope, s), "bn_bwd_reduce")
    _lib.check(lib.b200_bn_bwd_apply(_p(z), _p(da), _p(mi), _p(gamma), _p(beta), _p(sums), _p(dz), npix, c, slope,
                                     1 if use_batch_stats else 0, s), "bn_bwd_apply")
    return dz, dgamma, dbeta


def maxpool2x2(x):
    require_device(x, "maxpool2x2")
    N, H, W, Cc = x.shape
    y = torch.empty(N, H // 2, W // 2, Cc, dtype=BF16, device=x.device)
    _lib.check(lib.b200_maxpool2x2(_p(x), _p(y), N, H, W, Cc, stream_ptr()), "maxpool2x2")
    return y


def pixel_shuffle2(z, act=0, slope=0.2):
    require_device(z, "pixel_shuffle2")
    N, H, W, C4 = z.shape
    y = torch.empty(N, 2 * H, 2 * W, C4 // 4, dtype=BF16, device=z.device)
    _lib.check(lib.b200_pixel_shuffle2(_p(z), _p(y), N, H, W, C4 // 4, int(act), float(slope), stream_ptr()),
               "pixel_shuffle2")
    return y


def pixel_unshuffle2(dy):
    require_device(dy, "pixel_unshuffle2")
    N, H2, W2, Cc = dy.shape
    dz = torch.empty(N, H2 // 2, W2 // 2, 4 * Cc, dtype=BF16, device=dy.device)
    _lib.check(lib.b200_pixel_unshuffle2(_p(dy), _p(dz), N, H2 // 2, W2 // 2, Cc, stream_ptr()), "pixel_unshuffle2")
    return dz


def maxpool2x2_backward(x, dy):
    require_device(x, "maxpool2x2_backward")
    N, H, W, Cc = x.shape
    dx = torch.empty_like(x)
    _lib.check(lib.b200_maxpool2x2_bwd(_p(x), _p(dy), _p(dx), N, H, W, Cc, stream_ptr()), "maxpool2x2_bwd")
    return dx


def sumpool2x2_mask(dy, mask_up=None, slope=0.2):
    require_device(dy, "sumpool2x2_mask")
    N, H2, W2, Cc = dy.shape
    dx = torch.empty(N, H2 // 2, W2 // 2, Cc, dtype=BF16, device=dy.device)
    _lib.check(lib.b200_sumpool2x2_mask(_p(dy), _p(mask_up), _p(dx), N, H2 // 2, W2 // 2, Cc, slope, stream_ptr()),
               "sumpool2x2_mask")
    return dx


def l1_loss_with_grad(a, b, weight=1.0):
    require_device(a, "l1_loss")
    assert a.shape == b.shape and a.dtype == b.dtype and a.is_contiguous() and b.is_contiguous()
    loss = torch.empty(1, dtype=torch.float32, device=a.device)
    grad = torch.empty_like(a)
    fn = lib.b200_l1_loss_f32 if a.dtype == torch.float32 else lib.b200_l1_loss_bf16
    _lib.check(fn(_p(a), _p(b), _p(loss), _p(grad), a.numel(), float(weight), stream_ptr()), "l1_loss")
    return loss[0], grad


def to_flat(x_dense, c_total=None, coff=0):
    require_device(x_dense, "to_flat")
    N, H, W, Cc = x_dense.shape
    ct = Cc if c_total is None else c_total
    out = torch.zeros(N, H + 2, W + 2, ct, dtype=BF16, device=x_dense.device)
    _lib.check(lib.b200_pad_copy(_p(out), ct, coff, _p(x_dense), Cc, 0, N, H, W, Cc, stream_ptr()), "pad_copy")
    return out


def from_flat(x_flat, coff=0, c=None, add=None):
    require_device(x_flat, "from_flat")
    N, Hp, Wp, Ct = x_flat.shape
    c = Ct - coff if c is None else c
    out = torch.empty(N, Hp - 2, Wp - 2, c, dtype=BF16, device=x_flat.device)
    _lib.check(lib.b200_unpad_add(_p(out), c, _p(x_flat), Ct, coff, _p(add), add.shape[3] if add is not None else 8,
                                  N, Hp - 2, Wp - 2, c, stream_ptr()), "unpad_add")
    return out


def conv3x3_flat(x_flat, w_oihw, bias=None, dgrad=False, cin_off=0, out=None, cout_off=0, out_mode=0, act=0,
                 slope=0.2, alpha=1.0, res1=None, res1_coff=0, beta1=0.0, res2=None, res2_coff=0, beta2=0.0,
                 res_nch=0, accumulate=False, mask=None, mask_coff=0, mask_lo=0, mask_hi=0, mask_slope=0.2):
    require_device(x_flat, "conv3x3_flat")
    N, Hp, Wp, Cx = x_flat.shape
    h, w = Hp - 2, Wp - 2
    Cout, Cin, kh, kw = w_oihw.shape
    assert kh == 3 and kw == 3
    K, Nout = (Cout, Cin) if dgrad else (Cin, Cout)
    wp = pack_weight(w_oihw, 1 if dgrad else 0)
    taps = taps_dgrad_s1(3, 1) if dgrad else taps_conv(3, 1)
    if out is None:
        shape = {0: (N, Hp, Wp, Nout), 1: (N, h, w, Nout), 2: (N, 2 * h, 2 * w, Nout)}[out_mode]
        out = torch.zeros(*shape, dtype=BF16, device=x_flat.device)
    d = make_flat_desc(N, h, w, Cx, cin_off, K, out.shape[3], cout_off, Nout, taps, 9, wp.shape[1], wp.shape[2],
                       out_mode=out_mode, alpha=alpha, act=act, slope=slope, beta1=beta1, beta2=beta2,
                       res_nch=res_nch, res1_c=res1.shape[3] if res1 is not None else 0, res1_coff=res1_coff,
                       res2_c=res2.shape[3] if res2 is not None else 0, res2_coff=res2_coff,
                       accumulate=1 if accumulate else 0, mask_c=mask.shape[3] if mask is not None else 0,
                       mask_coff=mask_coff, mask_lo=mask_lo, mask_hi=mask_hi, mask_slope=mask_slope)
    b = bias.detach().float().contiguous() if bias is not None else None
    _lib.check(lib.b200_conv3x3_flat(C.byref(d), _p(x_flat), None, _p(wp), _p(b), _p(res1), _p(res2), _p(mask), _p(out),
                                     stream_ptr()), "conv3x3_flat")
    return out
```

Before: 40.37 million.

## Fuse BatchNorm+LeakyReLU stats and apply into one cooperative kernel with grid barrier

Replaces the separate BN stats/finalize and apply kernels (forward) and the reduce/apply pair (backward) with a single cooperative kernel per direction. A software grid barrier separates the reduction, per-channel finalize and apply phases. When the per-block slice fits, z and da are kept in shared memory so the apply phase does not read them from global memory a second time. This removes kernel launches and a second pass over activations. In exchange, the grid is capped to what can be co-resident, and the barrier uses a reserved counter word.

Measured after the change: 41.16 million, median of 6. 1.9% higher.

```diff
diff --git a/include/trainner_b200.h b/include/trainner_b200.h
--- a/include/trainner_b200.h
+++ b/include/trainner_b200.h
@@ -187,15 +187,13 @@
 int b200_bn_partials_finalize(const float* part, int32_t rows, float* stats, float* mean_invstd,
                               float* running_mean, float* running_var, int64_t npix, int32_t c, float momentum,
                               float eps, b200_stream_t stream);
-int b200_bn_apply_lrelu(const void* z, const float* mean_invstd, const float* gamma,
-                        const float* beta, void* a, int64_t npix, int32_t c, float slope,
-                        b200_stream_t stream);
-int b200_bn_bwd_reduce(const void* z, const void* da, const float* mean_invstd,
-                       const float* gamma, const float* beta, float* sums, float* dgamma, float* dbeta,
-                       int64_t npix, int32_t c, float slope, b200_stream_t stream);
-int b200_bn_bwd_apply(const void* z, const void* da, const float* mean_invstd, const float* gamma,
-                      const float* beta, const float* sums, void* dz, int64_t npix, int32_t c, float slope,
-                      int32_t use_batch_stats, b200_stream_t stream);
+int b200_bn_lrelu_fwd(const void* z, const float* conv_part, int32_t conv_rows, float* stats, float* mean_invstd,
+                      float* running_mean, float* running_var, const float* gamma, const float* beta, void* a,
+                      int64_t npix, int32_t c, float momentum, float eps, float slope, int32_t batch_stats,
+                      b200_stream_t stream);
+int b200_bn_lrelu_bwd(const void* z, const void* da, const float* mean_invstd, const float* gamma,
+                      const float* beta, float* sums, float* dgamma, float* dbeta, void* dz, int64_t npix,
+                      int32_t c, float slope, int32_t use_batch_stats, b200_stream_t stream);
 
 int b200_maxpool2x2(const void* x, void* y, int32_t n, int32_t h, int32_t w, int32_t c,
                     b200_stream_t stream);
diff --git a/trainner_b200/_lib.py b/trainner_b200/_lib.py
--- a/trainner_b200/_lib.py
+++ b/trainner_b200/_lib.py
@@ -129,9 +129,8 @@
     "b200_bn_stats_finalize": [_P, _P, _P, _P, _P, _L, _I, _F, _F, _P],
     "b200_bn_partials_finalize": [_P, _I, _P, _P, _P, _P, _L, _I, _F, _F, _P],
     "b200_bn_finalize_multi": [_P, _I, _I, _P],
-    "b200_bn_apply_lrelu": [_P, _P, _P, _P, _P, _L, _I, _F, _P],
-    "b200_bn_bwd_reduce": [_P, _P, _P, _P, _P, _P, _P, _P, _L, _I, _F, _P],
-    "b200_bn_bwd_apply": [_P, _P, _P, _P, _P, _P, _P, _L, _I, _F, _I, _P],
+    "b200_bn_lrelu_fwd": [_P, _P, _I, _P, _P, _P, _P, _P, _P, _P, _L, _I, _F, _F, _F, _I, _P],
+    "b200_bn_lrelu_bwd": [_P, _P, _P, _P, _P, _P, _P, _P, _P, _L, _I, _F, _I, _P],
     "b200_maxpool2x2": [_P, _P, _I, _I, _I, _I, _P],
     "b200_maxpool2x2_bwd": [_P, _P, _P, _I, _I, _I, _I, _P],
     "b200_sumpool2x2_mask": [_P, _P, _P, _I, _I, _I, _I, _F, _P],
diff --git a/trainner_b200/csrc/common.cu b/trainner_b200/csrc/common.cu
--- a/trainner_b200/csrc/common.cu
+++ b/trainner_b200/csrc/common.cu
@@ -71,7 +71,7 @@
 int det_scratch(DetScratch* out, size_t floats_needed, int counters_needed) {
   static std::mutex mu;
   static DetScratch per_dev[64] = {};
-  if (floats_needed > kDetFloats || counters_needed > kDetCounters)
+  if (floats_needed > kDetFloats || counters_needed > kGridBarrierWord)
     return set_error("deterministic-reduction scratch too small: need %zu floats / %d counters", floats_needed,
                      counters_needed);
   int dev = 0;
diff --git a/trainner_b200/csrc/common.cuh b/trainner_b200/csrc/common.cuh
--- a/trainner_b200/csrc/common.cuh
+++ b/trainner_b200/csrc/common.cuh
@@ -63,6 +63,7 @@
 };
 constexpr size_t kDetFloats = 16u << 20;
 constexpr int kDetCounters = 8192;
+constexpr int kGridBarrierWord = kDetCounters - 2;
 int det_scratch(DetScratch* out, size_t floats_needed, int counters_needed);
 
 inline cudaStream_t as_stream(b200_stream_t s) { return reinterpret_cast<cudaStream_t>(s); }
@@ -131,6 +132,26 @@
   }
   return true;
 }
+
+__device__ __forceinline__ void grid_barrier(unsigned* bar) {
+  __syncthreads();
+  if (threadIdx.x == 0) {
+    const unsigned gen = *reinterpret_cast<volatile unsigned*>(bar + 1);
+    __threadfence();
+    if (atomicAdd(bar, 1u) == gridDim.x - 1) {
+      atomicExch(bar, 0u);
+      __threadfence();
+      atomicAdd(bar + 1, 1u);
+    } else {
+      unsigned g;
+      do {
+        asm volatile("ld.acquire.gpu.global.u32 %0, [%1];" : "=r"(g) : "l"(bar + 1) : "memory");
+      } while (g == gen);
+    }
+    __threadfence();
+  }
+  __syncthreads();
+}
 #endif
 
 }
diff --git a/trainner_b200/csrc/elementwise.cu b/trainner_b200/csrc/elementwise.cu
--- a/trainner_b200/csrc/elementwise.cu
+++ b/trainner_b200/csrc/elementwise.cu
@@ -1,3 +1,5 @@
+#include <mutex>
+
 #include "common.cuh"
 
 namespace b200 {
@@ -48,67 +50,36 @@
   }
 }
 
-template <int MODE>
-__global__ void bn_reduce_kernel(const __nv_bfloat16* __restrict__ z,
-                                 const __nv_bfloat16* __restrict__ da,
-                                 const float* __restrict__ mean_invstd,
-                                 const float* __restrict__ gamma, const float* __restrict__ beta,
-                                 float* __restrict__ sums, long long npix, int c, float slope,
-                                 float* __restrict__ part, unsigned* __restrict__ counter,
-                                 float* __restrict__ dgamma, float* __restrict__ dbeta,
-                                 float* __restrict__ fin_mean_invstd, float* __restrict__ running_mean,
-                                 float* __restrict__ running_var, float momentum, float eps) {
+__global__ void bn_stats_kernel(const __nv_bfloat16* __restrict__ z, float* __restrict__ sums, long long npix, int c,
+                                float* __restrict__ part, unsigned* __restrict__ counter,
+                                float* __restrict__ fin_mean_invstd, float* __restrict__ running_mean,
+                                float* __restrict__ running_var, float momentum, float eps) {
   pdl_trigger();
   pdl_wait();
   const int vec_per_pix = c / 8;
   const long long total_vec = npix * vec_per_pix;
   const long long stride = (long long)gridDim.x * blockDim.x;
   long long i = (long long)blockIdx.x * blockDim.x + threadIdx.x;
-  const int cv = (int)(i % vec_per_pix) * 8;
   float s0[8], s1[8];
 #pragma unroll
   for (int j = 0; j < 8; ++j) s0[j] = s1[j] = 0.f;
-  float mu[8], is[8], ga[8], be[8];
-  if (MODE == 1) {
-#pragma unroll
-    for (int j = 0; j < 8; ++j) {
-      mu[j] = mean_invstd[cv + j];
-      is[j] = mean_invstd[c + cv + j];
-      ga[j] = gamma[cv + j];
-      be[j] = beta[cv + j];
-    }
-  }
   constexpr int U = 4;
   for (; i < total_vec; i += U * stride) {
-    uint4 zv[U], gv[U];
+    uint4 zv[U];
 #pragma unroll
     for (int u = 0; u < U; ++u) {
       const long long iu = i + u * stride;
       zv[u] = iu < total_vec ? reinterpret_cast<const uint4*>(z)[iu] : make_uint4(0, 0, 0, 0);
-      if (MODE == 1) gv[u] = iu < total_vec ? reinterpret_cast<const uint4*>(da)[iu] : make_uint4(0, 0, 0, 0);
     }
 #pragma unroll
     for (int u = 0; u < U; ++u) {
       if (i + u * stride >= total_vec) break;
       float f[8];
       unpack8(zv[u], f);
-      if (MODE == 0) {
-#pragma unroll
-        for (int j = 0; j < 8; ++j) {
-          s0[j] += f[j];
-          s1[j] = fmaf(f[j], f[j], s1[j]);
-        }
-      } else {
-        float g[8];
-        unpack8(gv[u], g);
-#pragma unroll
-        for (int j = 0; j < 8; ++j) {
-          const float zh = (f[j] - mu[j]) * is[j];
-          const float bn = fmaf(ga[j], zh, be[j]);
-          const float d = bn > 0.f ? g[j] : g[j] * slope;
-          s0[j] += d;
-          s1[j] = fmaf(d, zh, s1[j]);
-        }
+#pragma unroll
+      for (int j = 0; j < 8; ++j) {
+        s0[j] += f[j];
+        s1[j] = fmaf(f[j], f[j], s1[j]);
       }
     }
   }
@@ -126,17 +97,9 @@
     for (int q = ln; q < 256; q += vec_per_pix) t += sh[j * 256 + q];
     part[(size_t)k * gridDim.x + blockIdx.x] = t;
   }
-  const bool fin = det_reduce(part, part + (size_t)2 * c * gridDim.x, counter, gridDim.x, 2 * c, [&](int k, float t) {
-    sums[k] = t;
-    if (MODE == 1) {
-      if (k < c) {
-        if (dbeta) dbeta[k] += t;
-      } else if (dgamma) {
-        dgamma[k - c] += t;
-      }
-    }
-  });
-  if (MODE == 0 && fin && fin_mean_invstd) {
+  const bool fin = det_reduce(part, part + (size_t)2 * c * gridDim.x, counter, gridDim.x, 2 * c,
+                              [&](int k, float t) { sums[k] = t; });
+  if (fin && fin_mean_invstd) {
     __syncthreads();
     for (int ch = threadIdx.x; ch < c; ch += blockDim.x)
       bn_finalize_channel(sums, fin_mean_invstd, running_mean, running_var, npix, c, momentum, eps, ch);
@@ -150,6 +113,20 @@
   const int ch = blockIdx.x * blockDim.x + threadIdx.x;
   if (ch >= e.c) return;
   bn_finalize_channel(e.stats, e.mean_invstd, e.running_mean, e.running_var, e.npix, e.c, e.momentum, e.eps, ch);
+}
+
+__device__ __forceinline__ void warp_row_sums(const float* p0, const float* p1, int n, int lane, float& s0, float& s1) {
+  s0 = 0.f;
+  s1 = 0.f;
+  for (int i = lane; i < n; i += 32) {
+    s0 += __ldcg(p0 + i);
+    s1 += __ldcg(p1 + i);
+  }
+#pragma unroll
+  for (int o = 16; o > 0; o >>= 1) {
+    s0 += __shfl_xor_sync(0xffffffffu, s0, o);
+    s1 += __shfl_xor_sync(0xffffffffu, s1, o);
+  }
 }
 
 __global__ void __launch_bounds__(256) bn_partials_finalize_kernel(const float* __restrict__ part, int rows,
@@ -162,18 +139,8 @@
   pdl_wait();
   const int lane = threadIdx.x & 31, ch = blockIdx.x * 8 + (threadIdx.x >> 5);
   if (ch >= c) return;
-  float s0 = 0.f, s1 = 0.f;
-  const float* p0 = part + (size_t)ch * rows;
-  const float* p1 = part + (size_t)(c + ch) * rows;
-  for (int i = lane; i < rows; i += 32) {
-    s0 += p0[i];
-    s1 += p1[i];
-  }
-#pragma unroll
-  for (int o = 16; o > 0; o >>= 1) {
-    s0 += __shfl_xor_sync(0xffffffffu, s0, o);
-    s1 += __shfl_xor_sync(0xffffffffu, s1, o);
-  }
+  float s0, s1;
+  warp_row_sums(part + (size_t)ch * rows, part + (size_t)(c + ch) * rows, rows, lane, s0, s1);
   if (lane == 0) {
     stats[ch] = s0;
     stats[c + ch] = s1;
@@ -181,41 +148,184 @@
   }
 }
 
-template <int MODE>
-__global__ void bn_apply_kernel(const __nv_bfloat16* __restrict__ z,
-                                const __nv_bfloat16* __restrict__ da,
-                                const float* __restrict__ mean_invstd,
-                                const float* __restrict__ gamma, const float* __restrict__ beta,
-                                const float* __restrict__ sums, __nv_bfloat16* __restrict__ out,
-                                long long npix, int c, float slope, int use_batch_stats) {
-  pdl_trigger();
-  pdl_wait();
-  const int vec_per_pix = c / 8;
-  const long long total_vec = npix * vec_per_pix;
-  const long long stride = (long long)gridDim.x * blockDim.x;
-  long long i = (long long)blockIdx.x * blockDim.x + threadIdx.x;
-  const int cv = (int)(i % vec_per_pix) * 8;
-  float mu[8], is[8], ga[8], be[8], m0[8], m1[8];
-  const float inv_n = use_batch_stats ? 1.f / (float)npix : 0.f;
+constexpr int kBnThreads = 256;
+constexpr int kBnRedBytes = 16 * kBnThreads * (int)sizeof(float);
+constexpr int kBnSmemMax = 112 * 1024;
+constexpr int kBnMaxGrid = 148 * 2;
+
+struct BnFusedParams {
+  const __nv_bfloat16* z;
+  const __nv_bfloat16* da;
+  const float* gamma;
+  const float* beta;
+  float* mean_invstd;
+  float* sums;
+  const float* conv_part;
+  int conv_rows;
+  float* running_mean;
+  float* running_var;
+  float momentum, eps;
+  float* dgamma;
+  float* dbeta;
+  __nv_bfloat16* out;
+  float* part;
+  unsigned* bar;
+  long long npix;
+  int c;
+  int cache;
+  int tile_da;
+  int batch_stats;
+  float slope;
+};
+
+__device__ __forceinline__ float warp_grouped_sum(const float* row, int nblk, int lane) {
+  const int ngrp = det_groups(nblk);
+  float gs = 0.f;
+  if (lane < ngrp) {
+    const int g0 = lane * kDetGroup, members = min(kDetGroup, nblk - g0);
+    for (int i = 0; i < members; ++i) gs += __ldcg(row + g0 + i);
+  }
+  float t = 0.f;
+  for (int g = 0; g < ngrp; ++g) t += __shfl_sync(0xffffffffu, gs, g);
+  return t;
+}
+
+template <bool BWD>
+__global__ void __launch_bounds__(kBnThreads, 2) bn_lrelu_fused_kernel(const BnFusedParams p) {
+  pdl_trigger();
+  pdl_wait();
+  extern __shared__ __align__(16) uint4 bn_smem[];
+  float* red = reinterpret_cast<float*>(bn_smem);
+  uint4* tile = bn_smem + kBnRedBytes / 16;
+  const int c = p.c, vpp = c >> 3, tid = threadIdx.x;
+  const long long total_vec = p.npix * vpp;
+  const long long stride = (long long)gridDim.x * kBnThreads;
+  const long long i0 = (long long)blockIdx.x * kBnThreads + tid;
+  const int cv = (int)(i0 % vpp) * 8;
+  const uint4* zg = reinterpret_cast<const uint4*>(p.z);
+  const uint4* dg = reinterpret_cast<const uint4*>(p.da);
+  constexpr int U = 4;
+  float mu[8], is[8], ga[8], be[8];
 #pragma unroll
   for (int j = 0; j < 8; ++j) {
-    mu[j] = mean_invstd[cv + j];
-    is[j] = mean_invstd[c + cv + j];
-    ga[j] = gamma[cv + j];
-    be[j] = beta[cv + j];
-    if (MODE == 1) {
-      m0[j] = sums[cv + j] * inv_n;
-      m1[j] = sums[c + cv + j] * inv_n;
-    }
-  }
-  constexpr int U = 2;
-  for (; i < total_vec; i += U * stride) {
+    ga[j] = p.gamma[cv + j];
+    be[j] = p.beta[cv + j];
+    if (BWD) {
+      mu[j] = p.mean_invstd[cv + j];
+      is[j] = p.mean_invstd[c + cv + j];
+    }
+  }
+  const bool from_z = BWD || (p.batch_stats && !p.conv_part);
+  const bool use_tile = from_z && p.cache;
+  if (from_z) {
+    float s0[8], s1[8];
+#pragma unroll
+    for (int j = 0; j < 8; ++j) s0[j] = s1[j] = 0.f;
+    int e = 0;
+    for (long long i = i0; i < total_vec; i += U * stride, e += U) {
+      uint4 zv[U], gv[U];
+#pragma unroll
+      for (int u = 0; u < U; ++u) {
+        const long long iu = i + u * stride;
+        zv[u] = iu < total_vec ? zg[iu] : make_uint4(0, 0, 0, 0);
+        if (BWD) gv[u] = iu < total_vec ? dg[iu] : make_uint4(0, 0, 0, 0);
+      }
+#pragma unroll
+      for (int u = 0; u < U; ++u) {
+        if (i + u * stride >= total_vec) break;
+        if (use_tile) {
+          tile[(e + u) * kBnThreads + tid] = zv[u];
+          if (BWD) tile[p.tile_da + (e + u) * kBnThreads + tid] = gv[u];
+        }
+        float f[8];
+        unpack8(zv[u], f);
+        if (!BWD) {
+#pragma unroll
+          for (int j = 0; j < 8; ++j) {
+            s0[j] += f[j];
+            s1[j] = fmaf(f[j], f[j], s1[j]);
+          }
+        } else {
+          float g[8];
+          unpack8(gv[u], g);
+#pragma unroll
+          for (int j = 0; j < 8; ++j) {
+            const float zh = (f[j] - mu[j]) * is[j];
+            const float bn = fmaf(ga[j], zh, be[j]);
+            const float d = bn > 0.f ? g[j] : g[j] * p.slope;
+            s0[j] += d;
+            s1[j] = fmaf(d, zh, s1[j]);
+          }
+        }
+      }
+    }
+#pragma unroll
+    for (int j = 0; j < 8; ++j) {
+      red[j * kBnThreads + tid] = s0[j];
+      red[(8 + j) * kBnThreads + tid] = s1[j];
+    }
+    __syncthreads();
+    for (int k = tid; k < 2 * c; k += kBnThreads) {
+      const int which = k / c, ch = k - which * c;
+      const int ln = ch >> 3, j = (ch & 7) + 8 * which;
+      float t = 0.f;
+      for (int q = ln; q < kBnThreads; q += vpp) t += red[j * kBnThreads + q];
+      p.part[(size_t)k * gridDim.x + blockIdx.x] = t;
+    }
+    grid_barrier(p.bar);
+  }
+  if (BWD || p.batch_stats) {
+    const int lane = tid & 31, nw = kBnThreads / 32;
+    for (int ch = blockIdx.x * nw + (tid >> 5); ch < c; ch += gridDim.x * nw) {
+      float s0, s1;
+      if (from_z) {
+        s0 = warp_grouped_sum(p.part + (size_t)ch * gridDim.x, gridDim.x, lane);
+        s1 = warp_grouped_sum(p.part + (size_t)(c + ch) * gridDim.x, gridDim.x, lane);
+      } else {
+        warp_row_sums(p.conv_part + (size_t)ch * p.conv_rows, p.conv_part + (size_t)(c + ch) * p.conv_rows,
+                      p.conv_rows, lane, s0, s1);
+      }
+      if (lane == 0) {
+        p.sums[ch] = s0;
+        p.sums[c + ch] = s1;
+        if (BWD) {
+          if (p.dbeta) p.dbeta[ch] += s0;
+          if (p.dgamma) p.dgamma[ch] += s1;
+        } else {
+          bn_finalize_channel(p.sums, p.mean_invstd, p.running_mean, p.running_var, p.npix, c, p.momentum, p.eps, ch);
+        }
+      }
+    }
+    grid_barrier(p.bar);
+  }
+  float m0[8], m1[8];
+  const float inv_n = p.batch_stats ? 1.f / (float)p.npix : 0.f;
+#pragma unroll
+  for (int j = 0; j < 8; ++j) {
+    if (BWD) {
+      m0[j] = __ldcg(p.sums + cv + j) * inv_n;
+      m1[j] = __ldcg(p.sums + c + cv + j) * inv_n;
+    } else {
+      mu[j] = __ldcg(p.mean_invstd + cv + j);
+      is[j] = __ldcg(p.mean_invstd + c + cv + j);
+    }
+  }
+  uint4* og = reinterpret_cast<uint4*>(p.out);
+  int e = 0;
+  for (long long i = i0; i < total_vec; i += U * stride, e += U) {
     uint4 zv[U], gv[U];
 #pragma unroll
     for (int u = 0; u < U; ++u) {
       const long long iu = i + u * stride;
-      zv[u] = iu < total_vec ? reinterpret_cast<const uint4*>(z)[iu] : make_uint4(0, 0, 0, 0);
-      if (MODE == 1) gv[u] = iu < total_vec ? reinterpret_cast<const uint4*>(da)[iu] : make_uint4(0, 0, 0, 0);
+      if (iu >= total_vec) {
+        zv[u] = gv[u] = make_uint4(0, 0, 0, 0);
+      } else if (use_tile) {
+        zv[u] = tile[(e + u) * kBnThreads + tid];
+        if (BWD) gv[u] = tile[p.tile_da + (e + u) * kBnThreads + tid];
+      } else {
+        zv[u] = zg[iu];
+        if (BWD) gv[u] = dg[iu];
+      }
     }
 #pragma unroll
     for (int u = 0; u < U; ++u) {
@@ -223,11 +333,11 @@
       if (iu >= total_vec) break;
       float f[8], o[8];
       unpack8(zv[u], f);
-      if (MODE == 0) {
+      if (!BWD) {
 #pragma unroll
         for (int j = 0; j < 8; ++j) {
           const float bn = fmaf(ga[j], (f[j] - mu[j]) * is[j], be[j]);
-          o[j] = bn > 0.f ? bn : bn * slope;
+          o[j] = bn > 0.f ? bn : bn * p.slope;
         }
       } else {
         float g[8];
@@ -236,11 +346,11 @@
         for (int j = 0; j < 8; ++j) {
           const float zh = (f[j] - mu[j]) * is[j];
           const float bn = fmaf(ga[j], zh, be[j]);
-          const float d = bn > 0.f ? g[j] : g[j] * slope;
+          const float d = bn > 0.f ? g[j] : g[j] * p.slope;
           o[j] = ga[j] * is[j] * (d - m0[j] - zh * m1[j]);
         }
       }
-      reinterpret_cast<uint4*>(out)[iu] = pack8(o);
+      og[iu] = pack8(o);
     }
   }
 }
@@ -510,12 +620,11 @@
   B200_REQUIRE(mean_invstd != nullptr, "b200_bn_stats_finalize: mean_invstd is required");
   B200_REQUIRE(c % 8 == 0 && c <= 2048 && 256 % (c / 8) == 0,
                "b200_bn_stats_finalize: c/8 must be a power of two <= 256 (c=%d)", c);
-  const int grid = bn_grid(npix, c, 4, 148 * 2);
+  const int grid = bn_grid(npix, c, 4, kBnMaxGrid);
   DetScratch ds;
   if (det_scratch(&ds, (size_t)(grid + det_groups(grid)) * 2 * c, 1 + det_groups(grid))) return 1;
-  ::b200::launch_kernel(bn_reduce_kernel<0>, grid, 256, 16 * 256 * sizeof(float), as_stream(stream),
-      (const bf16*)z, nullptr, nullptr, nullptr, nullptr, stats, (long long)npix, c, 0.f, ds.part, ds.counters, nullptr, nullptr,
-      mean_invstd, running_mean, running_var, momentum, eps);
+  ::b200::launch_kernel(bn_stats_kernel, grid, 256, 16 * 256 * sizeof(float), as_stream(stream),
+      (const bf16*)z, stats, (long long)npix, c, ds.part, ds.counters, mean_invstd, running_mean, running_var, momentum, eps);
   B200_LAUNCH_CHECK();
   return 0;
 }
@@ -539,37 +648,115 @@
   return 0;
 }
 
-int b200_bn_apply_lrelu(const void* z, const float* mean_invstd, const float* gamma,
-                        const float* beta, void* a, int64_t npix, int32_t c, float slope,
-                        b200_stream_t stream) {
-  B200_REQUIRE(c % 8 == 0, "b200_bn_apply_lrelu: c must be a multiple of 8");
-  ::b200::launch_kernel(bn_apply_kernel<0>, bn_grid(npix, c, 2), 256, 0, as_stream(stream), 
-      (const bf16*)z, nullptr, mean_invstd, gamma, beta, nullptr, (bf16*)a, npix, c, slope, 1);
-  B200_LAUNCH_CHECK();
-  return 0;
-}
-
-int b200_bn_bwd_reduce(const void* z, const void* da, const float* mean_invstd, const float* gamma,
-                       const float* beta, float* sums, float* dgamma, float* dbeta, int64_t npix, int32_t c,
-                       float slope, b200_stream_t stream) {
-  B200_REQUIRE(c % 8 == 0 && c <= 2048 && 256 % (c / 8) == 0, "b200_bn_bwd_reduce: c/8 must be a power of two <= 256 (c=%d)", c);
-  const int grid = bn_grid(npix, c, 4, 148 * 2);
+}
+
+namespace {
+
+template <bool BWD>
+int bn_fused_max_grid(int* out) {
+  static std::mutex mu;
+  static int cache[64] = {0};
+  B200_ENSURE_SMEM(bn_lrelu_fused_kernel<BWD>, kBnSmemMax);
+  int dev = 0;
+  B200_CHECK_CUDA(cudaGetDevice(&dev));
+  B200_REQUIRE(dev >= 0 && dev < 64, "bn_lrelu: device index %d out of range", dev);
+  std::lock_guard<std::mutex> g(mu);
+  if (cache[dev] == 0) {
+    int per_sm = 0;
+    B200_CHECK_CUDA(cudaOccupancyMaxActiveBlocksPerMultiprocessor(&per_sm, bn_lrelu_fused_kernel<BWD>, kBnThreads,
+                                                                  kBnSmemMax));
+    B200_REQUIRE(per_sm >= 1, "bn_lrelu: the fused kernel does not fit on an SM");
+    cache[dev] = per_sm * sm_count();
+  }
+  *out = cache[dev];
+  return 0;
+}
+
+template <bool BWD>
+int bn_fused_launch(BnFusedParams& p, const char* name, b200_stream_t stream) {
+  B200_REQUIRE(p.c % 8 == 0 && p.c <= 2048 && kBnThreads % (p.c / 8) == 0,
+               "%s: c/8 must be a power of two <= 256 (c=%d)", name, p.c);
+  B200_REQUIRE(p.npix > 0, "%s: empty tensor", name);
+  int max_grid = 0;
+  if (bn_fused_max_grid<BWD>(&max_grid)) return 1;
+  const int grid = bn_grid(p.npix, p.c, 4, kBnMaxGrid);
+  B200_REQUIRE(grid <= max_grid, "%s: %d blocks are not co-resident on this device (%d)", name, grid, max_grid);
+  const bool from_z = BWD || (p.batch_stats && !p.conv_part);
+  const long long stride = (long long)grid * kBnThreads;
+  const long long per_thread = (p.npix * (p.c / 8) + stride - 1) / stride;
+  const long long tile_bytes = per_thread * kBnThreads * 16 * (BWD ? 2 : 1);
+  p.cache = from_z && tile_bytes <= kBnSmemMax - kBnRedBytes;
+  p.tile_da = (int)(per_thread * kBnThreads);
+  const size_t smem = kBnRedBytes + (p.cache ? (size_t)tile_bytes : 0);
   DetScratch ds;
-  if (det_scratch(&ds, (size_t)(grid + det_groups(grid)) * 2 * c, 1 + det_groups(grid))) return 1;
-  ::b200::launch_kernel(bn_reduce_kernel<1>, grid, 256, 16 * 256 * sizeof(float), as_stream(stream), 
-      (const bf16*)z, (const bf16*)da, mean_invstd, gamma, beta, sums, npix, c, slope, ds.part, ds.counters, dgamma, dbeta,
-      nullptr, nullptr, nullptr, 0.f, 0.f);
-  B200_LAUNCH_CHECK();
-  return 0;
-}
-
-int b200_bn_bwd_apply(const void* z, const void* da, const float* mean_invstd, const float* gamma,
-                      const float* beta, const float* sums, void* dz, int64_t npix, int32_t c, float slope,
+  if (det_scratch(&ds, (size_t)2 * p.c * grid, 0)) return 1;
+  p.part = ds.part;
+  p.bar = ds.counters + kGridBarrierWord;
+  cudaLaunchConfig_t cfg = {};
+  cfg.gridDim = dim3(grid);
+  cfg.blockDim = dim3(kBnThreads);
+  cfg.dynamicSmemBytes = smem;
+  cfg.stream = as_stream(stream);
+  cudaLaunchAttribute attr[1];
+  attr[0].id = cudaLaunchAttributeCooperative;
+  attr[0].val.cooperative = 1;
+  cfg.attrs = attr;
+  cfg.numAttrs = 1;
+  B200_CHECK_CUDA(cudaLaunchKernelEx(&cfg, bn_lrelu_fused_kernel<BWD>, (const BnFusedParams)p));
+  g_launches.fetch_add(1);
+  return 0;
+}
+
+}
+
+extern "C" {
+
+int b200_bn_lrelu_fwd(const void* z, const float* conv_part, int32_t conv_rows, float* stats, float* mean_invstd,
+                      float* running_mean, float* running_var, const float* gamma, const float* beta, void* a,
+                      int64_t npix, int32_t c, float momentum, float eps, float slope, int32_t batch_stats,
+                      b200_stream_t stream) {
+  B200_REQUIRE(z && mean_invstd && gamma && beta && a, "b200_bn_lrelu_fwd: null argument");
+  B200_REQUIRE(!batch_stats || stats, "b200_bn_lrelu_fwd: stats is required with batch statistics");
+  B200_REQUIRE(!conv_part || conv_rows > 0, "b200_bn_lrelu_fwd: conv_rows must be positive");
+  BnFusedParams p = {};
+  p.z = (const bf16*)z;
+  p.gamma = gamma;
+  p.beta = beta;
+  p.mean_invstd = mean_invstd;
+  p.sums = stats;
+  p.conv_part = conv_part;
+  p.conv_rows = conv_rows;
+  p.running_mean = running_mean;
+  p.running_var = running_var;
+  p.momentum = momentum;
+  p.eps = eps;
+  p.out = (bf16*)a;
+  p.npix = npix;
+  p.c = c;
+  p.batch_stats = batch_stats ? 1 : 0;
+  p.slope = slope;
+  return bn_fused_launch<false>(p, "b200_bn_lrelu_fwd", stream);
+}
+
+int b200_bn_lrelu_bwd(const void* z, const void* da, const float* mean_invstd, const float* gamma, const float* beta,
+                      float* sums, float* dgamma, float* dbeta, void* dz, int64_t npix, int32_t c, float slope,
                       int32_t use_batch_stats, b200_stream_t stream) {
-  ::b200::launch_kernel(bn_apply_kernel<1>, bn_grid(npix, c, 2), 256, 0, as_stream(stream), 
-      (const bf16*)z, (const bf16*)da, mean_invstd, gamma, beta, sums, (bf16*)dz, npix, c, slope, (int)use_batch_stats);
-  B200_LAUNCH_CHECK();
-  return 0;
+  B200_REQUIRE(z && da && mean_invstd && gamma && beta && sums && dz, "b200_bn_lrelu_bwd: null argument");
+  BnFusedParams p = {};
+  p.z = (const bf16*)z;
+  p.da = (const bf16*)da;
+  p.gamma = gamma;
+  p.beta = beta;
+  p.mean_invstd = const_cast<float*>(mean_invstd);
+  p.sums = sums;
+  p.dgamma = dgamma;
+  p.dbeta = dbeta;
+  p.out = (bf16*)dz;
+  p.npix = npix;
+  p.c = c;
+  p.batch_stats = use_batch_stats ? 1 : 0;
+  p.slope = slope;
+  return bn_fused_launch<true>(p, "b200_bn_lrelu_bwd", stream);
 }
 
 int b200_maxpool2x2(const void* x, void* y, int32_t n, int32_t h, int32_t w, int32_t c,
diff --git a/trainner_b200/engine_d.py b/trainner_b200/engine_d.py
--- a/trainner_b200/engine_d.py
+++ b/trainner_b200/engine_d.py
@@ -82,15 +82,12 @@
                     if ctx.stat_part[i] is None:
                         ctx.stat_part[i] = torch.empty(2 * L.cout * rows, dtype=torch.float32, device=dev)
                     add_igemm_stats(f, d, ctx.A[i], L.w_fwd, L.bias, ctx.Z[i], ctx.stat_part[i])
-                    f.add(lib.b200_bn_partials_finalize, P(ctx.stat_part[i]), rows, P(ctx.stats[i]), P(ctx.mi[i]),
-                          P(bn.running_mean), P(bn.running_var), npix, L.cout, float(bn.momentum), float(bn.eps))
                 else:
                     add_igemm(f, d, ctx.A[i], L.w_fwd, L.bias, y=ctx.Z[i])
-                if train and not rows:
-                    f.add(lib.b200_bn_stats_finalize, P(ctx.Z[i]), P(ctx.stats[i]), P(ctx.mi[i]),
-                          P(bn.running_mean), P(bn.running_var), npix, L.cout, float(bn.momentum), float(bn.eps))
-                f.add(lib.b200_bn_apply_lrelu, P(ctx.Z[i]), P(ctx.mi[i]), P(bn.weight), P(bn.bias),
-                      P(ctx.A[i + 1]), npix, L.cout, SL)
+                f.add(lib.b200_bn_lrelu_fwd, P(ctx.Z[i]), P(ctx.stat_part[i]) if rows else None, rows,
+                      P(ctx.stats[i]), P(ctx.mi[i]), P(bn.running_mean) if train else None,
+                      P(bn.running_var) if train else None, P(bn.weight), P(bn.bias), P(ctx.A[i + 1]), npix, L.cout,
+                      float(bn.momentum), float(bn.eps), SL, 1 if train else 0)
             f.add(lib.b200_nhwc_bf16_to_nchw_f32, P(ctx.A[-1]), P(ctx.feat), N, cl, ctx.hf, ctx.hf, cl, 0)
             return f
 
@@ -128,11 +125,9 @@
             L, bn = self.layers[i]
             hi, ho = ctx.dims[i]
             npix = N * ho * ho
-            b.add(lib.b200_bn_bwd_reduce, P(ctx.Z[i]), P(ctx.dA[i + 1]), P(ctx.mi[i]), P(bn.weight), P(bn.bias),
-                  P(ctx.sums[i]), P(g(bn.weight)) if wgrad else None, P(g(bn.bias)) if wgrad else None, npix, L.cout,
-                  SL)
-            b.add(lib.b200_bn_bwd_apply, P(ctx.Z[i]), P(ctx.dA[i + 1]), P(ctx.mi[i]), P(bn.weight), P(bn.bias),
-                  P(ctx.sums[i]), P(ctx.dZ[i]), npix, L.cout, SL, 1 if train else 0)
+            b.add(lib.b200_bn_lrelu_bwd, P(ctx.Z[i]), P(ctx.dA[i + 1]), P(ctx.mi[i]), P(bn.weight), P(bn.bias),
+                  P(ctx.sums[i]), P(g(bn.weight)) if wgrad else None, P(g(bn.bias)) if wgrad else None, P(ctx.dZ[i]),
+                  npix, L.cout, SL, 1 if train else 0)
             if wgrad:
                 add_wgrad(b, N, hi, hi, L.cin, 0, L.cin, ho, ho, L.cout, 0, L.cout, L.kh, L.stride, L.pad, 1.0,
                           ctx.A[i], ctx.dZ[i], g(L.weight), g(L.bias))
diff --git a/trainner_b200/ops.py b/trainner_b200/ops.py
--- a/trainner_b200/ops.py
+++ b/trainner_b200/ops.py
@@ -144,9 +144,8 @@
     mi = torch.empty(2 * c, dtype=torch.float32, device=z.device)
     a = torch.empty_like(z)
     s = stream_ptr()
-    _lib.check(lib.b200_bn_stats_finalize(_p(z), _p(stats), _p(mi), _p(running_mean), _p(running_var), npix, c,
-                                          momentum, eps, s), "bn_stats_finalize")
-    _lib.check(lib.b200_bn_apply_lrelu(_p(z), _p(mi), _p(gamma), _p(beta), _p(a), npix, c, slope, s), "bn_apply")
+    _lib.check(lib.b200_bn_lrelu_fwd(_p(z), None, 0, _p(stats), _p(mi), _p(running_mean), _p(running_var), _p(gamma),
+                                     _p(beta), _p(a), npix, c, momentum, eps, slope, 1, s), "bn_lrelu_fwd")
     return a, mi
 
 
@@ -159,10 +158,8 @@
     dgamma = torch.zeros(c, dtype=torch.float32, device=z.device)
     dbeta = torch.zeros(c, dtype=torch.float32, device=z.device)
     s = stream_ptr()
-    _lib.check(lib.b200_bn_bwd_reduce(_p(z), _p(da), _p(mi), _p(gamma), _p(beta), _p(sums), _p(dgamma), _p(dbeta), npix,
-                                      c, slope, s), "bn_bwd_reduce")
-    _lib.check(lib.b200_bn_bwd_apply(_p(z), _p(da), _p(mi), _p(gamma), _p(beta), _p(sums), _p(dz), npix, c, slope,
-                                     1 if use_batch_stats else 0, s), "bn_bwd_apply")
+    _lib.check(lib.b200_bn_lrelu_bwd(_p(z), _p(da), _p(mi), _p(gamma), _p(beta), _p(sums), _p(dgamma), _p(dbeta), _p(dz),
+                                     npix, c, slope, 1 if use_batch_stats else 0, s), "bn_lrelu_bwd")
     return dz, dgamma, dbeta
 
 
```
